# ChristianSteger/HORAYZON

Hardware: AMD Instinct MI355X
Metric: grid_cells_per_s (horizon_gridded, 360 azimuths, 3601^2 SRTM-like tile) (higher is better)
Workload: dtype f32

## Files before the change

### horayzon_amd/csrc/hz_api.hip

```cpp
#include "hz_internal.h"
#include <cmath>
#include <cstring>
#include <cstdlib>
#include <string>
#include <vector>
#include <limits>
#include <mutex>
#include <utility>
#include <thread>
#include <atomic>

namespace hz {

static thread_local std::string g_error;

int set_error(int code, const char *fmt, ...) {
    char buf[1024];
    va_list ap;
    va_start(ap, fmt);
    vsnprintf(buf, sizeof(buf), fmt, ap);
    va_end(ap);
    g_error = buf;
    return code;
}

bool is_device_ptr(const void *p) {
    if (!p) return false;
    hipPointerAttribute_t attr;
    const hipError_t e = hipPointerGetAttributes(&attr, p);
    if (e != hipSuccess) { (void)hipGetLastError(); return false; }
    return attr.type == hipMemoryTypeDevice || attr.type == hipMemoryTypeManaged;
}

template <typename T>
struct DevIn {
    const T *dev = nullptr;
    void *owned = nullptr;
    ~DevIn() { if (owned) (void)hipFree(owned); }
    int bind(const T *src, size_t count, hipStream_t st) {
        if (!src || count == 0) { dev = nullptr; return HZ_OK; }
        if (is_device_ptr(src)) { dev = src; return HZ_OK; }
        HZ_HIP(hipMalloc(&owned, count * sizeof(T)));
        HZ_HIP(hipMemcpyAsync(owned, src, count * sizeof(T), hipMemcpyHostToDevice, st));
        dev = static_cast<const T *>(owned);
        return HZ_OK;
    }
};

template <typename T>
struct DevOut {
    T *dev = nullptr;
    T *host = nullptr;
    void *owned = nullptr;
    size_t count = 0;
    ~DevOut() { if (owned) (void)hipFree(owned); }
    int bind(T *dst, size_t n) {
        count = n;
        if (!dst || n == 0) { dev = nullptr; return HZ_OK; }
        if (is_device_ptr(dst)) { dev = dst; return HZ_OK; }
        HZ_HIP(hipMalloc(&owned, n * sizeof(T)));
        dev = static_cast<T *>(owned); host = dst;
        return HZ_OK;
    }
    int finish(hipStream_t st) {
        if (host && count) HZ_HIP(hipMemcpyAsync(host, dev, count * sizeof(T), hipMemcpyDeviceToHost, st));
        return HZ_OK;
    }
};

static int select_device(int device) {
    int n = 0;
    if (hipGetDeviceCount(&n) != hipSuccess || n <= 0) {
        (void)hipGetLastError();
        return set_error(HZ_ERR_NODEV, "no HIP device available (libhorayzon_hip needs an MI355X / gfx950 GPU)");
    }
    if (device < 0 || device >= n) return set_error(HZ_ERR_ARG, "device %d out of range (%d devices)", device, n);
    HZ_HIP(hipSetDevice(device));
    return HZ_OK;
}

static inline float deg2rad_f(float ang) { return (float)(((double)ang / 180.0) * M_PI); }

struct HostTables {
    std::vector<float> azim_sin, azim_cos, elev_ang, elev_sin, elev_cos;
    std::vector<int> mid_idx;
    int elev_num = 0;
    float hori_acc = 0, low = 0, up = 0;
};

static void build_tables(int azim_num, float hori_acc_deg, float low_deg, HostTables &t) {
    float elev_ang_up_lim = 89.98;
    t.hori_acc = deg2rad_f(hori_acc_deg);
    t.low = deg2rad_f(low_deg);
    t.up = deg2rad_f(elev_ang_up_lim);
    t.azim_sin.resize((size_t)azim_num); t.azim_cos.resize((size_t)azim_num);
    float ang;
    for (int i = 0; i < azim_num; i++) {
        ang = (float)(((2 * M_PI) / azim_num) * i);
        t.azim_sin[(size_t)i] = sinf(ang);
        t.azim_cos[(size_t)i] = cosf(ang);
    }
    const double step = (double)t.hori_acc / 5.0;
    t.elev_num = (int)ceil((double)(t.up - t.low) / step) + 1;
    const size_t n = (size_t)std::max(t.elev_num, 0);
    t.elev_ang.resize(n); t.elev_sin.resize(n); t.elev_cos.resize(n);
    for (int i = 0; i < t.elev_num; i++) {
        ang = (float)((double)t.up - step * (double)i);
        t.elev_ang[(size_t)(t.elev_num - i - 1)] = ang;
        t.elev_sin[(size_t)(t.elev_num - i - 1)] = sinf(ang);
        t.elev_cos[(size_t)(t.elev_num - i - 1)] = cosf(ang);
    }
    t.mid_idx.assign(2 * (n > 0 ? n : 1), 0);
    for (int i = 0; i + 10 < t.elev_num; i++) {
        const float es = (float)((double)(t.elev_ang[(size_t)i] + t.elev_ang[(size_t)i + 10]) / 2.0);
        const int mid = (int)roundf((float)((double)(es - t.low) / step));
        t.mid_idx[2 * (size_t)i] = mid;
        const float ev = t.elev_ang[(size_t)std::min(std::max(mid, 0), t.elev_num - 1)];
        memcpy(&t.mid_idx[2 * (size_t)i + 1], &ev, sizeof(float));
    }
}

static int parse_alg(const char *s, int *alg) {
    if (s && strcmp(s, "discrete_sampling") == 0) { *alg = 0; return HZ_OK; }
    if (s && strcmp(s, "binary_search") == 0) { *alg = 1; return HZ_OK; }
    if (s && strcmp(s, "guess_constant") == 0) { *alg = 2; return HZ_OK; }
    return set_error(HZ_ERR_ARG, "invalid input argument for ray_algorithm");
}

static int check_geom(const char *s) {
    if (s && (strcmp(s, "triangle") == 0 || strcmp(s, "quad") == 0 || strcmp(s, "grid") == 0)) return HZ_OK;
    return set_error(HZ_ERR_ARG, "invalid input argument for geom_type");
}

static std::mutex g_stream_mu;
static std::vector<std::pair<int, hipStream_t>> g_stream_pool;

static int stream_acquire(int device, hipStream_t *st) {
    {
        std::lock_guard<std::mutex> lk(g_stream_mu);
        for (size_t i = 0; i < g_stream_pool.size(); i++)
            if (g_stream_pool[i].first == device) {
                *st = g_stream_pool[i].second;
                g_stream_pool.erase(g_stream_pool.begin() + (long)i);
                return HZ_OK;
            }
    }
    const hipError_t e = hipStreamCreateWithFlags(st, hipStreamNonBlocking);
    if (e != hipSuccess) return set_error(HZ_ERR_HIP, "hipStreamCreate failed: %s", hipGetErrorString(e));
    return HZ_OK;
}

static void stream_release(int device, hipStream_t st) {
    if (!st) return;
    (void)hipStreamSynchronize(st);
    std::lock_guard<std::mutex> lk(g_stream_mu);
    g_stream_pool.emplace_back(device, st);
}

static int scene_new(int device, Scene **out) {
    int rc = select_device(device);
    if (rc) return rc;
    Scene *sc = new Scene();
    sc->device = device;
    if ((rc = stream_acquire(device, &sc->stream))) { delete sc; return rc; }
    *out = sc;
    return HZ_OK;
}

static void scene_free(Scene *sc) {
    if (!sc) return;
    (void)hipSetDevice(sc->device);
    stream_release(sc->device, sc->stream);
    if (sc->near_buf) (void)hipFree(sc->near_buf);
    if (sc->left_buf) (void)hipFree(sc->left_buf);
    if (sc->owns_blob && sc->blob) (void)hipFree(sc->blob);
    delete sc;
}

struct Terrain {
    int device = 0;
    Scene *scene = nullptr;
    bool owns_scene = false;
    int offset_0 = 0, offset_1 = 0, dim_in_0 = 0, dim_in_1 = 0;
    void *tilt = nullptr, *norm = nullptr, *enl = nullptr, *elev = nullptr, *mask = nullptr;
    double *refrac_fac = nullptr;
    bool own_tilt = false, own_norm = false, own_enl = false, own_elev = false, own_mask = false;
    float fill = 0, ang_max = 89.0f;
    int refrac = 0;
    int count_work = 0;
    unsigned long long *counters = nullptr;
    float *sun_dev = nullptr;
    size_t sun_cap = 0;
    hipStream_t stream = nullptr;
    bool initialised = false;
};

static void terrain_release_arrays(Terrain *t) {
    (void)hipSetDevice(t->device);
    if (t->own_tilt && t->tilt) (void)hipFree(t->tilt);
    if (t->own_norm && t->norm) (void)hipFree(t->norm);
    if (t->own_enl && t->enl) (void)hipFree(t->enl);
    if (t->own_elev && t->elev) (void)hipFree(t->elev);
    if (t->own_mask && t->mask) (void)hipFree(t->mask);
    if (t->refrac_fac) { (void)hipFree(t->refrac_fac); t->refrac_fac = nullptr; }
    t->tilt = t->norm = t->enl = t->elev = t->mask = nullptr;
    t->own_tilt = t->own_norm = t->own_enl = t->own_elev = t->own_mask = false;
    if (t->counters) { (void)hipFree(t->counters); t->counters = nullptr; }
    if (t->sun_dev) { (void)hipFree(t->sun_dev); t->sun_dev = nullptr; t->sun_cap = 0; }
    if (t->owns_scene && t->scene) scene_free(t->scene);
    t->scene = nullptr; t->owns_scene = false; t->initialised = false;
}

static int persist(const void *src, size_t bytes, hipStream_t st, void **dst, bool *own) {
    if (is_device_ptr(src)) { *dst = const_cast<void *>(src); *own = false; return HZ_OK; }
    HZ_HIP(hipMalloc(dst, bytes ? bytes : 16));
    *own = true;
    HZ_HIP(hipMemcpyAsync(*dst, src, bytes, hipMemcpyHostToDevice, st));
    return HZ_OK;
}

struct HostPinner {
    std::vector<std::pair<char *, size_t>> regions;
    std::vector<std::pair<char *, size_t>> planned;
    std::atomic<int> done{0};
    std::atomic<bool> failed{false};
    std::thread worker;
    int device = 0;
    void start(int dev, char *base, const std::vector<size_t> &chunk_bytes) {
        device = dev;
        const uintptr_t page = 4096;
        size_t total = 0;
        for (size_t b : chunk_bytes) total += b;
        if (total < ((size_t)8 << 20)) return;
        const uintptr_t first = reinterpret_cast<uintptr_t>(base);
        const uintptr_t last_page = (first + total) & ~(page - 1);
        uintptr_t lo = (first + page - 1) & ~(page - 1);
        uintptr_t cur = first;
        for (size_t k = 0; k < chunk_bytes.size(); k++) {
            cur += chunk_bytes[k];
            const uintptr_t hi = std::min(cur & ~(page - 1), last_page);
            regions.emplace_back(reinterpret_cast<char *>(lo), hi > lo ? (size_t)(hi - lo) : 0);
            lo = std::max(lo, hi);
        }
        planned = regions;
        worker = std::thread([this]() {
            (void)hipSetDevice(device);
            for (size_t k = 0; k < regions.size(); k++) {
                if (!failed.load() && regions[k].second &&
                    hipHostRegister(regions[k].first, regions[k].second, hipHostRegisterDefault) != hipSuccess) {
                    (void)hipGetLastError();
                    regions[k].second = 0;
                    failed.store(true);
                } else if (failed.load()) {
                    regions[k].second = 0;
                }
                done.store((int)k + 1, std::memory_order_release);
            }
        });
    }
    std::vector<size_t> cuts_for(const char *dst, size_t bytes) const {
        std::vector<size_t> cuts;
        int need = 0;
        for (size_t k = 0; k < planned.size(); k++) {
            const char *lo = planned[k].first, *hi = lo + planned[k].second;
            if (planned[k].second && hi > dst && lo < dst + bytes) need = (int)k + 1;
        }
        while (done.load(std::memory_order_acquire) < need) std::this_thread::yield();
        for (int k = 0; k < need; k++) {
            const char *lo = planned[(size_t)k].first, *hi = lo + planned[(size_t)k].second;
            if (planned[(size_t)k].second == 0) continue;
            if (lo > dst && lo < dst + bytes) cuts.push_back((size_t)(lo - dst));
            if (hi > dst && hi < dst + bytes) cuts.push_back((size_t)(hi - dst));
        }
        std::sort(cuts.begin(), cuts.end());
        cuts.erase(std::unique(cuts.begin(), cuts.end()), cuts.end());
        return cuts;
    }
    void finish() {
        if (worker.joinable()) worker.join();
        for (auto &r : regions) if (r.second) (void)hipHostUnregister(r.first);
        regions.clear();
    }
    ~HostPinner() { finish(); }
};

struct NearMonitor {
    int device = 0;
    hipStream_t st_mon = nullptr;
    hipEvent_t ready = nullptr, done = nullptr;
    void *buf = nullptr;
    size_t buf_bytes = 0;
    unsigned long long *cnt = nullptr;
    bool active = false;
    int launch(const Scene *sc, const HorizonArgs &a, int n, int seed, hipStream_t st) {
        device = sc->device;
        const int nb = horizon_num_blocks(a);
        std::vector<int> pick;
        for (int b = 0; b < nb; b++) {
            uint32_t h = (uint32_t)b * 2654435761u + (uint32_t)seed * 40503u;
            h ^= h >> 15; h *= 2246822519u; h ^= h >> 13;
            if (h % (uint32_t)n == 0u) pick.push_back(b);
        }
        if (pick.empty()) return HZ_OK;
        int rc;
        if (!st_mon && (rc = stream_acquire(device, &st_mon))) return rc;
        if (!ready) { HZ_HIP(hipEventCreateWithFlags(&ready, hipEventDisableTiming)); HZ_HIP(hipEventCreateWithFlags(&done, hipEventDisableTiming)); }
        const size_t cbytes = HZ_CNT_N * sizeof(unsigned long long) + HZ_REDO_CAP * sizeof(int);
        const size_t row_bytes = ((size_t)a.azim_num * sizeof(float) + 255) & ~(size_t)255;
        const size_t need = cbytes + row_bytes + pick.size() * sizeof(int);
        if (need > buf_bytes) {
            if (buf) { (void)hipFree(buf); buf = nullptr; buf_bytes = 0; }
            HZ_HIP(hipMalloc(&buf, need + need / 4));
            buf_bytes = need + need / 4;
        }
        cnt = (unsigned long long *)buf;
        float *scratch = (float *)((char *)buf + cbytes);
        int *d_list = (int *)((char *)buf + cbytes + row_bytes);
        HZ_HIP(hipEventRecord(ready, st));
        HZ_HIP(hipStreamWaitEvent(st_mon, ready, 0));
        HZ_HIP(hipMemsetAsync(buf, 0, cbytes, st_mon));
        HZ_HIP(hipMemcpyAsync(d_list, pick.data(), pick.size() * sizeof(int), hipMemcpyHostToDevice, st_mon));
        HZ_HIP(hipStreamSynchronize(st_mon));
        HorizonArgs v = a;
        v.count_work = 1; v.verify_near = 1; v.level_stack = 1;
        v.scratch_row = scratch;
        v.counters = cnt; v.tile_list = d_list; v.n_list = (int)pick.size();
        if ((rc = horizon_launch(sc, v, st_mon, nullptr))) return rc;
        HZ_HIP(hipEventRecord(done, st_mon));
        active = true;
        return HZ_OK;
    }
    int collect(hipStream_t st, unsigned long long *verified, unsigned long long *violations) {
        unsigned long long c2[HZ_CNT_N] = {0};
        HZ_HIP(hipStreamWaitEvent(st, done, 0));
        HZ_HIP(hipMemcpyAsync(c2, cnt, sizeof(c2), hipMemcpyDeviceToHost, st_mon));
        HZ_HIP(hipStreamSynchronize(st_mon));
        *verified += c2[21]; *violations += c2[10];
        active = false;
        return HZ_OK;
    }
    ~NearMonitor() {
        if (st_mon) { (void)hipSetDevice(device); stream_release(device, st_mon); }
        if (ready) (void)hipEventDestroy(ready);
        if (done) (void)hipEventDestroy(done);
        if (buf) (void)hipFree(buf);
    }
};

static void print_near_reasons(const unsigned *near_reasons) {
    unsigned h[20] = {0};
    if (hipMemcpy(h, near_reasons, sizeof(h), hipMemcpyDeviceToHost) != hipSuccess) { (void)hipGetLastError(); return; }
    static const char *nm[14] = {"frame", "vertex_on_axis", "edge_over_axis", "az_tolerance", "inplane_edge", "crossing_near_axis",
                                 "interval", "precision", "edge_on", "orientation", "origin_below", "axis_in_triangle", "window_or_mask",
                                 "bad_mesh_nearby"};
    fprintf(stderr, "hz near reasons: cells %u certified %u", h[0], h[1]);
    for (int b = 0; b < 14; b++) if (h[2 + b]) fprintf(stderr, " %s %u", nm[b], h[2 + b]);
    fprintf(stderr, " | tasks %u bins %u\n", h[16], h[17]);
}

static void print_reference_report(const Scene *sc, int alg, unsigned long long cells, unsigned long long rays, size_t slab_cells,
                                   int dim_in_0, int dim_in_1, int azim_num, double kernel_s, bool certificates_off, bool certificates_per_cell) {
    static const char *alg_name[3] = {"discrete_sampling", "binary search", "guess horizon from previous azimuth direction"};
    printf("Horizon detection algorithm: %s\n", alg_name[alg]);
    printf("Number of grid cells for which horizon is computed: %llu \n", cells);
    printf("Fraction of total number of grid cells: %g %%\n", (double)((float)cells / (float)slab_cells * 100.0f));
    printf("Total memory required for horizon output: %g GB\n",
           (double)(((float)dim_in_0 * (float)dim_in_1 * (float)azim_num * 4.0f) / 1.0e9f));
    printf("Ray tracing time: %g s\n", kernel_s);
    printf("Number of rays shot: %llu\n", rays);
    printf("Average number of rays per location and azimuth: %.2f \n",
           cells ? (double)((float)rays / (float)(cells * (unsigned long long)azim_num)) : 0.0);
    if (certificates_off)
        printf("Near-field certificates off: a DEM quad that is not part of a height field over the (x, y) plane, or a triangle "
               "of the outer simplified domain, is too large for the per-cell guard (results unaffected, slower)\n");
    else if (certificates_per_cell)
        printf("Near-field certificates per cell: %u DEM triangle(s) project onto the (x, y) plane collapsed or against the "
               "majority, %d outer-domain triangle(s); cells near them run without (results unaffected)\n", sc->hdr.n_flipped, sc->hdr.n_tin);
    fflush(stdout);
}

static int alloc_hori_chunk(int rows_all, size_t row_bytes, bool skip_hori, int fixed_rows, int *chunk_rows_out, void **buf) {
    size_t target = skip_hori ? ((size_t)16 << 30) : ((size_t)4 << 30);
    {
        size_t free_b = 0, total_b = 0;
        if (hipMemGetInfo(&free_b, &total_b) == hipSuccess) {
            if (!skip_hori) {
                const size_t all = (size_t)rows_all * row_bytes;
                const size_t parts = std::max<size_t>(1, (all + ((size_t)8 << 30) - 1) / ((size_t)8 << 30));
                if (free_b / 6 >= all / parts + row_bytes) target = std::max(target, all / parts + row_bytes);
            }
        } else (void)hipGetLastError();
    }
    const bool fixed = fixed_rows > 0;
    for (;;) {
        int chunk_rows = rows_all;
        if (fixed) chunk_rows = std::min(chunk_rows, fixed_rows);
        else {
            chunk_rows = (int)std::max<size_t>(16, std::min<size_t>((size_t)chunk_rows, target / row_bytes));
            const int n_ch = (rows_all + chunk_rows - 1) / chunk_rows;
            chunk_rows = std::min(chunk_rows, std::max(16, ((rows_all + n_ch - 1) / n_ch + 15) / 16 * 16));
        }
        chunk_rows = std::min(chunk_rows, rows_all);
        *chunk_rows_out = chunk_rows;
        if (hipMalloc(buf, (size_t)chunk_rows * row_bytes) == hipSuccess) return HZ_OK;
        (void)hipGetLastError();
        *buf = nullptr;
        if (fixed || target <= ((size_t)1 << 30)) return set_error(HZ_ERR_HIP, "hipMalloc of the horizon chunk (%zu bytes) failed", (size_t)chunk_rows * row_bytes);
        target >>= 1;
    }
}

static int near_prepass(const Scene *sc, NearArgs &na, hipStream_t st, float *ms_near) {
    const size_t cells = (size_t)(na.row_end - na.row_begin) * na.dim_in_1;
    const size_t idx_bytes = (cells * (size_t)na.azim_num * 2 + 255) & ~(size_t)255;
    const size_t need = idx_bytes + cells * 4;
    if (sc->near_bytes < need) {
        if (sc->near_buf) (void)hipFree(sc->near_buf);
        sc->near_buf = nullptr; sc->near_bytes = 0;
        if (hipMalloc(&sc->near_buf, need) != hipSuccess) return set_error(HZ_ERR_HIP, "hipMalloc of the near-field certificates failed");
        sc->near_bytes = need;
    }
    na.near_idx = (unsigned short *)sc->near_buf;
    na.near_r = (float *)((char *)sc->near_buf + idx_bytes);
    hipEvent_t n0 = nullptr, n1 = nullptr;
    if (hipEventCreate(&n0) != hipSuccess || hipEventCreate(&n1) != hipSuccess) {
        if (n0) (void)hipEventDestroy(n0);
        return set_error(HZ_ERR_HIP, "hipEventCreate failed");
    }
    (void)hipEventRecord(n0, st);
    const int rc = near_launch(sc, na, st);
    (void)hipEventRecord(n1, st);
    if (!rc) {
        (void)hipEventSynchronize(n1);
        float mn = 0.0f;
        (void)hipEventElapsedTime(&mn, n0, n1);
        *ms_near += mn;
    }
    (void)hipEventDestroy(n0); (void)hipEventDestroy(n1);
    return rc;
}

static int plan_leftover(const Scene *sc, const hz_opts *opts, int rows_max, int dim_in_1, int left_t[HZ_LEFT_LEVELS], HorizonArgs &a) {
    int n_left_launches = 0;
    for (int l = 0; l < HZ_LEFT_LEVELS; l++) left_t[l] = 0;
    const int pack = opts ? opts->left_min : 0;
    const unsigned upack = pack == 0 ? HZ_LEFT_DEFAULT : (pack < 0 ? 0u : (unsigned)pack);
    for (int l = 0; l < HZ_LEFT_LEVELS; l++) {
        left_t[l] = (int)std::min((upack >> (8 * l)) & 0xffu, 56u);
        if (left_t[l] == 0) break;
        n_left_launches = l + 1;
    }
    if ((opts && opts->count_work) || n_left_launches == 0) return 0;
    const TileMap tm = make_tile_map((rows_max + 15) / 16, (dim_in_1 + 15) / 16);
    unsigned long long units = (unsigned long long)tm.per_xcd * 8ull * 4ull;
    unsigned long long total = 0, cap_max = 0;
    for (int l = 0; l < n_left_launches; l++) {
        unsigned long long cap = ((units * (unsigned long long)left_t[l] + 63ull) & ~63ull) + 64ull;
        if (opts && opts->left_cap_test > 0) cap = std::min<unsigned long long>(cap, ((unsigned long long)opts->left_cap_test + 63ull) & ~63ull);
        a.left_base[l] = (unsigned)total; a.left_cap[l] = (unsigned)cap;
        total += cap; cap_max = std::max(cap_max, cap);
        units = cap / 64ull;
    }
    const size_t rec_bytes = (size_t)total * HZ_LEFT_WORDS * sizeof(unsigned);
    const size_t sort_words = 4 * (size_t)cap_max + sort_temp_elems((size_t)cap_max) + 64;
    const size_t need = rec_bytes + sort_words * sizeof(uint32_t);
    if (total >= (1ull << 31) || (unsigned long long)rows_max * (unsigned long long)dim_in_1 >= 0xffffffffull) return 0;
    if (sc->left_bytes < need) {
        if (sc->left_buf) (void)hipFree(sc->left_buf);
        sc->left_buf = nullptr; sc->left_bytes = 0;
        if (hipMalloc(&sc->left_buf, need) != hipSuccess) { (void)hipGetLastError(); sc->left_buf = nullptr; return 0; }
        sc->left_bytes = need;
    }
    a.left_sort = (uint32_t *)((char *)sc->left_buf + rec_bytes); a.left_cap_max = (unsigned)cap_max;
    return n_left_launches;
}

static int horizon_run(const Scene *sc, const float *vec_norm, const float *vec_north, int offset_0,
                       int offset_1, float *hori_buffer, int dim_in_0, int dim_in_1, int azim_num,
                       float dist_search, float hori_acc, const char *ray_algorithm,
                       float elev_ang_low_lim, const uint8_t *mask, float hori_fill, float ray_org_elev,
                       const hz_opts *opts, const hz_topo_out *topo, hz_stats *stats) {
    int alg = 2;
    int rc = parse_alg(ray_algorithm, &alg);
    if (rc) return rc;
    if (!vec_norm || !vec_north || !mask) return set_error(HZ_ERR_ARG, "vec_norm, vec_north and mask must not be NULL");
    if (dim_in_0 <= 0 || dim_in_1 <= 0 || azim_num <= 0) return set_error(HZ_ERR_ARG, "dim_in_0, dim_in_1 and azim_num must be positive");
    if (offset_0 < 0 || offset_1 < 0 || offset_0 + dim_in_0 > sc->hdr.d0 || offset_1 + dim_in_1 > sc->hdr.d1)
        return set_error(HZ_ERR_ARG, "inconsistency between input arguments dem_dim_0, dem_dim_1, offset_0, offset_1 and vec_norm");
    if (!(hori_acc > 0.0f) || hori_acc > 10.0f) return set_error(HZ_ERR_ARG, "limit of hori_acc (10 degree) is exceeded");
    const bool skip_hori = opts && opts->skip_hori;
    if (!hori_buffer && !skip_hori) return set_error(HZ_ERR_ARG, "hori_buffer is NULL");
    if (opts && opts->svf && !opts->vec_tilt) return set_error(HZ_ERR_ARG, "opts.svf needs opts.vec_tilt");
    if (opts && opts->svf && azim_num < 2) return set_error(HZ_ERR_ARG, "opts.svf needs azim_num >= 2");
    if (topo && topo->size != (int32_t)sizeof(hz_topo_out))
        return set_error(HZ_ERR_ARG, "topo.size is %d, expected sizeof(hz_topo_out) = %d", topo->size, (int)sizeof(hz_topo_out));
    const bool want_vsf = topo && topo->vsf, want_open = topo && topo->openness;
    if (want_vsf && !(opts && opts->vec_tilt)) return set_error(HZ_ERR_ARG, "topo.vsf needs opts.vec_tilt");
    if (want_vsf && azim_num < 2) return set_error(HZ_ERR_ARG, "topo.vsf needs azim_num >= 2");
    int row_begin = 0, row_end = dim_in_0;
    if (opts && !(opts->row_begin == 0 && opts->row_end == 0)) {
        row_begin = opts->row_begin;
        row_end = (opts->row_end == -1) ? dim_in_0 : opts->row_end;
        if (row_begin < 0 || row_end < 0 || row_end > dim_in_0 || row_begin > row_end)
            return set_error(HZ_ERR_ARG, "invalid row slab [%d, %d) for dim_in_0 = %d", opts->row_begin, opts->row_end, dim_in_0);
        if (row_begin == row_end) return HZ_OK;
    }
    HZ_HIP(hipSetDevice(sc->device));
    std::lock_guard<std::mutex> run_lock(sc->run_mu);
    hipStream_t st = sc->stream;
    Timer t_total; t_total.start();

    HostTables tb;
    build_tables(azim_num, hori_acc, elev_ang_low_lim, tb);
    if (tb.elev_num < 2) return set_error(HZ_ERR_ARG, "elevation table is empty (elev_ang_low_lim too high)");
    const float dist_m = (float)((double)dist_search * 1000.0);

    const size_t ncell = (size_t)dim_in_0 * dim_in_1;
    const size_t slab_cells = (size_t)(row_end - row_begin) * dim_in_1;
    Timer t_h2d; t_h2d.start();
    DevIn<float> d_norm, d_north, d_tilt, d_as, d_ac, d_ea, d_es, d_ec;
    DevIn<int> d_mid;
    DevIn<uint8_t> d_mask;
    const bool inputs_are_slab = opts && opts->inputs_are_slab;
    const size_t in_off = (size_t)row_begin * dim_in_1;
    const size_t src_off = inputs_are_slab ? 0 : in_off;
    (void)ncell;
    if ((rc = d_norm.bind(vec_norm + 3 * src_off, slab_cells * 3, st))) return rc;
    if ((rc = d_north.bind(vec_north + 3 * src_off, slab_cells * 3, st))) return rc;
    if ((rc = d_mask.bind(mask + src_off, slab_cells, st))) return rc;
    if ((opts && opts->svf) || want_vsf) if ((rc = d_tilt.bind(opts->vec_tilt + 3 * src_off, slab_cells * 3, st))) return rc;
    const float *norm0 = d_norm.dev - 3 * in_off, *north0 = d_north.dev - 3 * in_off;
    const uint8_t *mask0 = d_mask.dev - in_off;
    const float *tilt0 = d_tilt.dev ? d_tilt.dev - 3 * in_off : nullptr;
    if ((rc = d_as.bind(tb.azim_sin.data(), (size_t)azim_num, st))) return rc;
    if ((rc = d_ac.bind(tb.azim_cos.data(), (size_t)azim_num, st))) return rc;
    if ((rc = d_ea.bind(tb.elev_ang.data(), (size_t)tb.elev_num, st))) return rc;
    if ((rc = d_es.bind(tb.elev_sin.data(), (size_t)tb.elev_num, st))) return rc;
    if ((rc = d_ec.bind(tb.elev_cos.data(), (size_t)tb.elev_num, st))) return rc;
    if ((rc = d_mid.bind(tb.mid_idx.data(), tb.mid_idx.size(), st))) return rc;
    DevOut<float> d_hori, d_svf, d_vsf, d_open;
    DevIn<float> d_azim;
    const bool want_svf = opts && opts->svf;
    const bool want_topo = want_svf || want_vsf || want_open;
    const bool hori_is_slab = opts && opts->hori_is_slab;
    float *hori_slab_host = hori_buffer ? (hori_is_slab ? hori_buffer : hori_buffer + (size_t)row_begin * dim_in_1 * azim_num) : nullptr;
    float *hori_row0 = hori_slab_host ? hori_slab_host - (size_t)row_begin * dim_in_1 * azim_num : nullptr;
    float *svf_slab = want_svf ? (hori_is_slab ? opts->svf : opts->svf + (size_t)row_begin * dim_in_1) : nullptr;
    if ((rc = d_svf.bind(svf_slab, svf_slab ? slab_cells : 0))) return rc;
    float *vsf_slab = want_vsf ? (hori_is_slab ? topo->vsf : topo->vsf + (size_t)row_begin * dim_in_1) : nullptr;
    float *open_slab = want_open ? (hori_is_slab ? topo->openness : topo->openness + (size_t)row_begin * dim_in_1) : nullptr;
    if ((rc = d_vsf.bind(vsf_slab, vsf_slab ? slab_cells : 0))) return rc;
    if ((rc = d_open.bind(open_slab, open_slab ? slab_cells : 0))) return rc;
    int chunk_rows = row_end - row_begin;
    void *tmp_hori = nullptr, *tmp_hori2 = nullptr;
    size_t tmp_bytes = 0;
    struct TmpFree { void **p; ~TmpFree() { if (*p) (void)hipFree(*p); } } tmp_free{&tmp_hori}, tmp_free2{&tmp_hori2};
    const size_t row_bytes = (size_t)dim_in_1 * azim_num * 4;
    const bool stream_out = !skip_hori && !is_device_ptr(hori_slab_host);
    if (skip_hori || stream_out) {
        if (skip_hori && !want_topo) return set_error(HZ_ERR_ARG, "skip_hori without svf, vsf or openness: nothing to compute");
        if ((rc = alloc_hori_chunk(row_end - row_begin, row_bytes, skip_hori, (opts && opts->chunk_rows > 0) ? opts->chunk_rows : 0, &chunk_rows, &tmp_hori)))
            return rc;
        tmp_bytes = (size_t)chunk_rows * row_bytes;
        if (stream_out && chunk_rows < row_end - row_begin) { HZ_HIP(hipMalloc(&tmp_hori2, (size_t)chunk_rows * row_bytes)); tmp_bytes *= 2; }
    } else {
        if ((rc = d_hori.bind(hori_slab_host, slab_cells * (size_t)azim_num))) return rc;
    }
    std::vector<float> azim_h;
    if (want_topo) {
        azim_h.resize((size_t)azim_num);
        for (int i = 0; i < azim_num; i++) azim_h[(size_t)i] = (float)(((2 * M_PI) / azim_num) * i);
        if ((rc = d_azim.bind(azim_h.data(), (size_t)azim_num, st))) return rc;
    }
    DevIn<unsigned long long> d_cnt;
    unsigned long long zeros[HZ_CNT_N] = {0};
    void *cnt_dev = nullptr;
    HZ_HIP(hipMalloc(&cnt_dev, sizeof(zeros) + 2 * HZ_REDO_CAP * sizeof(int)));
    d_cnt.owned = cnt_dev;
    HZ_HIP(hipStreamSynchronize(st));
    const double h2d_s = t_h2d.stop();

    HorizonArgs a;
    a.vec_norm = norm0; a.vec_north = north0; a.mask = mask0;
    a.offset_0 = offset_0; a.offset_1 = offset_1; a.dim_in_0 = dim_in_0; a.dim_in_1 = dim_in_1;
    a.azim_num = azim_num; a.elev_num = tb.elev_num; a.alg = alg;
    a.hori_acc = tb.hori_acc; a.low = tb.low; a.up = tb.up; a.dist = dist_m;
    a.hori_fill = hori_fill; a.ray_org_elev = ray_org_elev;
    a.azim_sin = d_as.dev; a.azim_cos = d_ac.dev; a.elev_ang = d_ea.dev; a.elev_sin = d_es.dev; a.elev_cos = d_ec.dev;
    a.mid_idx = d_mid.dev;
    a.top_nodes = opts ? opts->top_nodes : -1;
    a.regroup = opts ? opts->regroup : -1;
    a.count_work = opts ? opts->count_work : 0;
    a.hit_cache = (opts && opts->no_hit_cache) ? 0 : 1;
    a.counters = (unsigned long long *)cnt_dev;
    const int near_opt = opts ? opts->no_near_skip : 0;
    const bool height_field = (sc->hdr.flags & HZ_BLOB_HEIGHT_FIELD) != 0;
    const bool bad_map = (sc->hdr.flags & HZ_BLOB_BAD_MAP) != 0;
    const bool use_near = near_opt <= 0 && (height_field || bad_map || near_opt < 0) &&
                          azim_num <= near_max_azim() && tb.elev_num <= 65534;
    a.near_idx = nullptr; a.near_r = nullptr; a.scratch_row = nullptr;
    a.tile_list = nullptr; a.n_list = 0;
    const int verify_n = (opts && opts->verify_near > 0) ? opts->verify_near : 0;
    a.verify_near = (opts && opts->count_work) ? verify_n : 0;
    float ms_near = 0.0f;

    unsigned long long cnt[16] = {0}, n_verified = 0, n_mon_violations = 0;
    NearMonitor mon;
    float ms = 0.0f, ms_svf = 0.0f;
    int fallbacks = 0;
    unsigned long long redo_blocks = 0, redo_groups = 0;

    struct Ev { hipEvent_t a = nullptr, b = nullptr, c = nullptr, d = nullptr, l = nullptr; };
    std::vector<Ev> evs;
    std::vector<size_t> ev_of;
    hipStream_t st_copy = nullptr;
    auto free_events = [&]() {
        for (auto &e : evs) {
            if (e.a) (void)hipEventDestroy(e.a);
            if (e.b) (void)hipEventDestroy(e.b);
            if (e.c) (void)hipEventDestroy(e.c);
            if (e.d) (void)hipEventDestroy(e.d);
            if (e.l) (void)hipEventDestroy(e.l);
        }
        if (st_copy) { stream_release(sc->device, st_copy); st_copy = nullptr; }
    };
    if (stream_out && (rc = stream_acquire(sc->device, &st_copy))) return rc;
    if (use_near) {
        const size_t cells = (size_t)std::min(chunk_rows, row_end - row_begin) * dim_in_1;
        const size_t need = ((cells * (size_t)azim_num * 2 + 255) & ~(size_t)255) + cells * 4;
        if (sc->near_bytes < need) {
            if (sc->near_buf) (void)hipFree(sc->near_buf);
            sc->near_buf = nullptr; sc->near_bytes = 0;
            if (hipMalloc(&sc->near_buf, need) != hipSuccess) { free_events(); return set_error(HZ_ERR_HIP, "hipMalloc of the near-field certificates failed"); }
            sc->near_bytes = need;
        }
    }
    int left_t[HZ_LEFT_LEVELS];
    const int n_left_launches = plan_leftover(sc, opts, std::min(chunk_rows, row_end - row_begin), dim_in_1, left_t, a);
    a.left_min = n_left_launches > 0 ? left_t[0] : 0;
    a.left_rec = n_left_launches > 0 ? (unsigned *)sc->left_buf : nullptr;
    a.left_regroup = (opts && (opts->left_tune & 0xff) > 0) ? (opts->left_tune & 0xff) : HZ_LEFT_REGROUP;
    a.left_key_shift = (opts && ((opts->left_tune >> 8) & 0xff) > 0) ? std::min(((opts->left_tune >> 8) & 0xff) - 1, 8) : HZ_LEFT_KEY_SHIFT;
    a.persist_grid = (opts && opts->persist_grid > 0) ? opts->persist_grid : 0;
    a.no_persist = (opts && opts->persist_grid < 0) ? 1 : 0;
    unsigned *near_reasons = nullptr;
    struct ReasonsFree { unsigned **p; ~ReasonsFree() { if (*p) (void)hipFree(*p); } } reasons_free{&near_reasons};
    if (use_near && opts && opts->verbose >= 2) {
        if (hipMalloc((void **)&near_reasons, 20 * sizeof(unsigned)) != hipSuccess) { (void)hipGetLastError(); near_reasons = nullptr; }
        else (void)hipMemsetAsync(near_reasons, 0, 20 * sizeof(unsigned), st);
    }
    HostPinner pinner;
    if (stream_out && !(opts && opts->no_host_pin)) {
        std::vector<size_t> cb;
        for (int rb = row_begin; rb < row_end; rb += chunk_rows) cb.push_back((size_t)(std::min(rb + chunk_rows, row_end) - rb) * row_bytes);
        pinner.start(sc->device, reinterpret_cast<char *>(hori_slab_host), cb);
    }
    auto copy_out = [&](int k) -> int {
        const int rb = row_begin + k * chunk_rows, re = std::min(rb + chunk_rows, row_end);
        const void *src = (k & 1) ? tmp_hori2 : tmp_hori;
        Ev &e = evs[ev_of[(size_t)k]];
        char *dst = reinterpret_cast<char *>(hori_row0 + (size_t)rb * dim_in_1 * azim_num);
        const size_t bytes = (size_t)(re - rb) * row_bytes;
        std::vector<size_t> cuts;
        if (!pinner.planned.empty()) cuts = pinner.cuts_for(dst, bytes);
        cuts.push_back(bytes);
        if (hipStreamWaitEvent(st_copy, e.c, 0) != hipSuccess)
            return set_error(HZ_ERR_HIP, "copy of the horizon chunk failed: %s", hipGetErrorString(hipGetLastError()));
        size_t from = 0;
        for (size_t to : cuts) {
            if (to > from && hipMemcpyAsync(dst + from, static_cast<const char *>(src) + from, to - from, hipMemcpyDeviceToHost, st_copy) != hipSuccess)
                return set_error(HZ_ERR_HIP, "copy of the horizon chunk failed: %s", hipGetErrorString(hipGetLastError()));
            from = to;
        }
        if (hipEventRecord(e.d, st_copy) != hipSuccess)
            return set_error(HZ_ERR_HIP, "copy of the horizon chunk failed: %s", hipGetErrorString(hipGetLastError()));
        return HZ_OK;
    };
    auto fail = [&](int code) { (void)hipStreamSynchronize(st); if (st_copy) (void)hipStreamSynchronize(st_copy); free_events(); return code; };
    int n_chunk = 0;
    unsigned long long left_cells = 0, left_again = 0;
    float ms_left = 0.0f;
    for (int rb = row_begin; rb < row_end; rb += chunk_rows, n_chunk++) {
        const int re = std::min(rb + chunk_rows, row_end);
        float *hori_chunk;
        if (stream_out) hori_chunk = (float *)((n_chunk & 1) ? tmp_hori2 : tmp_hori);
        else if (skip_hori) hori_chunk = (float *)tmp_hori;
        else hori_chunk = d_hori.dev + (size_t)(rb - row_begin) * dim_in_1 * azim_num;
        a.hori = hori_chunk - (size_t)rb * dim_in_1 * azim_num;
        a.row_begin = rb; a.row_end = re;
        if (use_near) {
            NearArgs na;
            na.vec_norm = norm0; na.vec_north = north0; na.mask = mask0;
            na.azim_sin = d_as.dev; na.azim_cos = d_ac.dev;
            na.offset_0 = offset_0; na.offset_1 = offset_1; na.dim_in_1 = dim_in_1; na.row_begin = rb; na.row_end = re;
            na.azim_num = azim_num; na.elev_num = tb.elev_num;
            na.ray_org_elev = ray_org_elev; na.hori_acc = tb.hori_acc; na.low = tb.low; na.up = tb.up;
            na.reasons = near_reasons;
            na.ignore_bad_map = near_opt < 0 ? 1 : 0;
            if ((rc = near_prepass(sc, na, st, &ms_near))) return fail(rc);
            a.near_idx = na.near_idx; a.near_r = na.near_r;
        }
        {
            Ev e;
            if (hipEventCreate(&e.a) != hipSuccess || hipEventCreate(&e.b) != hipSuccess || hipEventCreate(&e.c) != hipSuccess ||
                hipEventCreate(&e.d) != hipSuccess) {
                evs.push_back(e);
                return fail(set_error(HZ_ERR_HIP, "hipEventCreate failed"));
            }
            evs.push_back(e);
            ev_of.push_back(evs.size() - 1);
            if (hipMemcpyAsync(cnt_dev, zeros, sizeof(zeros), hipMemcpyHostToDevice, st) != hipSuccess)
                return fail(set_error(HZ_ERR_HIP, "counter reset failed"));
            if (stream_out && n_chunk >= 2) (void)hipStreamWaitEvent(st, evs[ev_of[(size_t)n_chunk - 2]].d, 0);
            a.level_stack = (sc->level_stack.load(std::memory_order_relaxed) != 0 || (opts && opts->level_stack > 0)) ? 1
                            : ((opts && opts->level_stack < 0) ? opts->level_stack : 0);
            (void)hipEventRecord(e.a, st);
            if (verify_n > 0 && !a.count_work && use_near) {
                if ((rc = mon.launch(sc, a, verify_n, rb, st))) return fail(rc);
            }
            auto launch_chunk = [&](int *safe_out) -> int {
                int r = horizon_launch(sc, a, st, safe_out);
                if (r || n_left_launches == 0) return r;
                if (!evs.back().l && hipEventCreate(&evs.back().l) != hipSuccess) return set_error(HZ_ERR_HIP, "hipEventCreate failed");
                (void)hipEventRecord(evs.back().l, st);
                for (int l = 1; l <= n_left_launches && !r; l++) {
                    if ((r = left_sort(a, l - 1, st))) break;
                    HorizonArgs b = a;
                    b.left_mode = l; b.left_min = l < n_left_launches ? left_t[l] : 0;
                    if (n_left_launches > 1) b.level_stack = 1;
                    b.tile_list = nullptr; b.n_list = 0;
                    r = horizon_launch(sc, b, st, nullptr);
                }
                return r;
            };
            int safe = 0;
            rc = launch_chunk(&safe);
            if (!rc && !safe) {
                unsigned long long cov[32] = {0};
                if (hipMemcpyAsync(cov, cnt_dev, sizeof(cov), hipMemcpyDeviceToHost, st) != hipSuccess ||
                    hipStreamSynchronize(st) != hipSuccess)
                    return fail(set_error(HZ_ERR_HIP, "horizon kernel failed: %s", hipGetErrorString(hipGetLastError())));
                const unsigned long long ov = cov[8], lov = cov[30];
                if (ov != 0 || lov != 0) {
                    const unsigned long long tiles = (unsigned long long)((re - rb + 7) / 8) * (unsigned long long)((dim_in_1 + 7) / 8);
                    fallbacks++;
                    a.level_stack = 1;
                    if (ov <= HZ_REDO_CAP && lov <= HZ_REDO_CAP && (ov + lov) * 4 <= tiles) {
                        redo_blocks += ov + lov; redo_groups += lov;
                        if (ov != 0) {
                            a.tile_list = reinterpret_cast<const int *>((unsigned long long *)cnt_dev + HZ_CNT_N);
                            a.n_list = (int)ov;
                            rc = horizon_launch(sc, a, st, &safe);
                            a.tile_list = nullptr; a.n_list = 0;
                        }
                        if (!rc && lov != 0) {
                            HorizonArgs b = a;
                            b.left_mode = 1; b.left_min = 0;
                            b.tile_list = reinterpret_cast<const int *>((unsigned long long *)cnt_dev + HZ_CNT_N) + HZ_REDO_CAP;
                            b.n_list = (int)lov;
                            rc = horizon_launch(sc, b, st, nullptr);
                        }
                    } else {
                        sc->level_stack.store(1, std::memory_order_relaxed);
                        if (hipMemcpyAsync(cnt_dev, zeros, sizeof(zeros), hipMemcpyHostToDevice, st) != hipSuccess)
                            return fail(set_error(HZ_ERR_HIP, "counter reset failed"));
                        (void)hipEventRecord(e.a, st);
                        rc = launch_chunk(&safe);
                    }
                }
            }
            if (!rc && mon.active) rc = mon.collect(st, &n_verified, &n_mon_violations);
            (void)hipEventRecord(e.b, st);
            if (!rc && want_topo) {
                const size_t o = (size_t)(rb - row_begin) * dim_in_1;
                const float *tilt_chunk = tilt0 ? tilt0 + 3 * (size_t)rb * dim_in_1 : nullptr;
                if (!want_vsf && !want_open)
                    rc = svf_launch(d_azim.dev, hori_chunk, tilt_chunk, re - rb, dim_in_1, azim_num, d_svf.dev + o, st);
                else
                    rc = topo_multi_launch(d_azim.dev, hori_chunk, tilt_chunk, re - rb, dim_in_1, azim_num,
                                           want_svf ? d_svf.dev + o : nullptr, want_vsf ? d_vsf.dev + o : nullptr,
                                           want_open ? d_open.dev + o : nullptr, st);
            }
            (void)hipEventRecord(e.c, st);
            if (!rc && stream_out && n_chunk >= 1) rc = copy_out(n_chunk - 1);
            if (rc) return fail(rc);
            unsigned long long c[HZ_CNT_N];
            if (hipMemcpyAsync(c, cnt_dev, sizeof(c), hipMemcpyDeviceToHost, st) != hipSuccess ||
                hipStreamSynchronize(st) != hipSuccess)
                return fail(set_error(HZ_ERR_HIP, "horizon kernel failed: %s", hipGetErrorString(hipGetLastError())));
            float m1 = 0.0f, m2 = 0.0f;
            (void)hipEventElapsedTime(&m1, e.a, e.b);
            (void)hipEventElapsedTime(&m2, e.b, e.c);
            ms += m1; ms_svf += m2;
            if (evs.back().l) { float m3 = 0.0f; (void)hipEventElapsedTime(&m3, evs.back().l, e.b); ms_left += m3; }
            for (int k = 0; k < 16; k++) cnt[k] += c[k];
            left_cells += c[28]; left_again += c[29];
            n_verified += c[21];
            if (a.count_work && opts && opts->verbose >= 3) {
                const unsigned long long t0 = ~c[20];
                fprintf(stderr, "hz xcd spans [ms] rows %d..%d:", rb, re);
                for (int x = 0; x < 8; x++) fprintf(stderr, " %.1f", c[12 + x] ? (double)(c[12 + x] - t0) * 1.0e-5 : 0.0);
                fprintf(stderr, "\n");
            }
        }
    }
    Timer t_d2h; t_d2h.start();
    if (stream_out) {
        rc = copy_out(n_chunk - 1);
        const hipError_t se = hipStreamSynchronize(st_copy);
        pinner.finish();
        if (!rc && se != hipSuccess) rc = set_error(HZ_ERR_HIP, "copy of the horizon failed: %s", hipGetErrorString(se));
        if (rc) { free_events(); return rc; }
    }
    free_events();
    HZ_HIP(hipGetLastError());
    if ((rc = d_hori.finish(st))) return rc;
    if ((rc = d_svf.finish(st))) return rc;
    if ((rc = d_vsf.finish(st))) return rc;
    if ((rc = d_open.finish(st))) return rc;
    HZ_HIP(hipStreamSynchronize(st));
    const double d2h_s = t_d2h.stop();

    if (stats) {
        stats->num_rays += cnt[0]; stats->guard_events += cnt[1];
        stats->nodes_visited += cnt[2]; stats->tris_tested += cnt[3]; stats->num_cells += cnt[4];
        stats->wave_node_iters += cnt[5]; stats->wave_leaf_iters += cnt[6]; stats->wave_refills += cnt[7];
        stats->t_h2d_s += h2d_s; stats->t_kernel_s += (double)ms * 1e-3; stats->t_svf_s += (double)ms_svf * 1e-3;
        stats->t_d2h_s += d2h_s;
        stats->t_total_s += t_total.stop();
        stats->elev_num = tb.elev_num; stats->bvh_height = sc->hdr.height; stats->scene_bytes = sc->hdr.total_bytes;
        stats->stack_fallbacks += (uint64_t)fallbacks; stats->stack_redo_blocks += redo_blocks; stats->left_redo_groups += redo_groups;
        stats->rays_shortened += cnt[9]; stats->near_violations += cnt[10] + n_mon_violations; stats->t_near_s += (double)ms_near * 1e-3;
        stats->guard_cells += cnt[11]; stats->near_verified += n_verified;
        stats->t_left_s += (double)ms_left * 1e-3; stats->left_cells += left_cells; stats->left_again += left_again;
        stats->scratch_bytes = (uint64_t)((use_near ? sc->near_bytes : 0) + (n_left_launches > 0 ? sc->left_bytes : 0) + tmp_bytes);
        stats->height_field = height_field ? 1 : 0; stats->near_used = use_near ? 1 : 0;
    }
    if (near_reasons) print_near_reasons(near_reasons);
    if (opts && opts->verbose)
        print_reference_report(sc, alg, cnt[4], cnt[0], slab_cells, dim_in_0, dim_in_1, azim_num, (double)ms * 1e-3,
                               !use_near && near_opt <= 0 && !height_field && !bad_map, use_near && bad_map);
    return HZ_OK;
}

static int locations_run(const Scene *sc, const float *coords, const float *vec_norm, const float *vec_north,
                         float *hori_buffer, float *hori_dist_buffer, int num_loc, int azim_num,
                         float dist_search, float hori_acc, const char *ray_algorithm, float elev_ang_low_lim,
                         const float *ray_org_elev, int hori_dist_out, const hz_opts *opts, hz_stats *stats) {
    int alg = 1;
    int rc = parse_alg(ray_algorithm, &alg);
    if (rc) return rc;
    if (hori_dist_out && alg == 2)
        return set_error(HZ_ERR_ARG, "horizon detection algorithm 'guess_constant' not implemented for horizon "
                                     "distance computation");
    if (!coords || !vec_norm || !vec_north || !ray_org_elev || !hori_buffer) return set_error(HZ_ERR_ARG, "NULL argument");
    if (hori_dist_out && !hori_dist_buffer) return set_error(HZ_ERR_ARG, "hori_dist_buffer is NULL");
    if (num_loc <= 0 || azim_num <= 0) return set_error(HZ_ERR_ARG, "num_loc and azim_num must be positive");
    if (!(hori_acc > 0.0f) || hori_acc > 10.0f) return set_error(HZ_ERR_ARG, "limit of hori_acc (10 degree) is exceeded");
    HZ_HIP(hipSetDevice(sc->device));
    std::lock_guard<std::mutex> run_lock(sc->run_mu);
    hipStream_t st = sc->stream;
    Timer t_total; t_total.start();
    HostTables tb;
    build_tables(azim_num, hori_acc, elev_ang_low_lim, tb);
    if (tb.elev_num < 2) return set_error(HZ_ERR_ARG, "elevation table is empty (elev_ang_low_lim too high)");
    Timer t_h2d; t_h2d.start();
    DevIn<float> d_co, d_norm, d_north, d_roe, d_as, d_ac, d_ea, d_es, d_ec;
    DevIn<int> d_mid;
    const size_t n = (size_t)num_loc;
    if ((rc = d_co.bind(coords, n * 3, st))) return rc;
    if ((rc = d_norm.bind(vec_norm, n * 3, st))) return rc;
    if ((rc = d_north.bind(vec_north, n * 3, st))) return rc;
    if ((rc = d_roe.bind(ray_org_elev, n, st))) return rc;
    if ((rc = d_as.bind(tb.azim_sin.data(), (size_t)azim_num, st))) return rc;
    if ((rc = d_ac.bind(tb.azim_cos.data(), (size_t)azim_num, st))) return rc;
    if ((rc = d_ea.bind(tb.elev_ang.data(), (size_t)tb.elev_num, st))) return rc;
    if ((rc = d_es.bind(tb.elev_sin.data(), (size_t)tb.elev_num, st))) return rc;
    if ((rc = d_ec.bind(tb.elev_cos.data(), (size_t)tb.elev_num, st))) return rc;
    if ((rc = d_mid.bind(tb.mid_idx.data(), tb.mid_idx.size(), st))) return rc;
    DevOut<float> d_hori, d_dist;
    if ((rc = d_hori.bind(hori_buffer, n * (size_t)azim_num))) return rc;
    if (d_hori.host) HZ_HIP(hipMemcpyAsync(d_hori.dev, hori_buffer, n * (size_t)azim_num * 4, hipMemcpyHostToDevice, st));
    if (hori_dist_out) {
        if ((rc = d_dist.bind(hori_dist_buffer, n * (size_t)azim_num))) return rc;
        if (d_dist.host) HZ_HIP(hipMemcpyAsync(d_dist.dev, hori_dist_buffer, n * (size_t)azim_num * 4, hipMemcpyHostToDevice, st));
    }
    DevIn<unsigned long long> d_cnt;
    unsigned long long zeros[8] = {0, 0, 0, 0, 0, 0, 0, 0};
    void *cnt_dev = nullptr;
    HZ_HIP(hipMalloc(&cnt_dev, sizeof(zeros)));
    d_cnt.owned = cnt_dev;
    HZ_HIP(hipMemcpyAsync(cnt_dev, zeros, sizeof(zeros), hipMemcpyHostToDevice, st));
    HZ_HIP(hipStreamSynchronize(st));
    const double h2d_s = t_h2d.stop();

    LocationsArgs a;
    a.coords = d_co.dev; a.vec_norm = d_norm.dev; a.vec_north = d_north.dev; a.ray_org_elev = d_roe.dev;
    a.hori = d_hori.dev; a.dist = d_dist.dev;
    a.num_loc = num_loc; a.azim_num = azim_num; a.elev_num = tb.elev_num; a.alg = alg; a.hori_dist_out = hori_dist_out;
    a.hori_acc = tb.hori_acc; a.low = tb.low; a.up = tb.up; a.dist_m = (float)((double)dist_search * 1000.0);
    a.azim_sin = d_as.dev; a.azim_cos = d_ac.dev; a.elev_ang = d_ea.dev; a.elev_sin = d_es.dev; a.elev_cos = d_ec.dev;
    a.mid_idx = d_mid.dev;
    a.counters = (unsigned long long *)cnt_dev;
    hipEvent_t e0, e1;
    HZ_HIP(hipEventCreate(&e0)); HZ_HIP(hipEventCreate(&e1));
    (void)hipEventRecord(e0, st);
    rc = locations_launch(sc, a, st);
    (void)hipEventRecord(e1, st);
    const hipError_t se = hipStreamSynchronize(st);
    float ms = 0.0f;
    (void)hipEventElapsedTime(&ms, e0, e1);
    (void)hipEventDestroy(e0); (void)hipEventDestroy(e1);
// ... 199 lines not shown
    if (!scene) return set_error(HZ_ERR_ARG, "scene is NULL");
    return locations_run(reinterpret_cast<const Scene *>(scene), coords, vec_norm, vec_north, hori_buffer,
                         hori_dist_buffer, num_loc, azim_num, dist_search, hori_acc, ray_algorithm,
                         elev_ang_low_lim, ray_org_elev, hori_dist_out, opts, stats);
}

int hz_horizon_locations(const float *vert_grid, int dem_dim_0, int dem_dim_1, const float *coords,
                         const float *vec_norm, const float *vec_north, float *hori_buffer,
                         float *hori_dist_buffer, int num_loc, int azim_num, float dist_search, float hori_acc,
                         const char *ray_algorithm, const char *geom_type, float elev_ang_low_lim,
                         const float *ray_org_elev, int hori_dist_out, const hz_opts *opts, hz_stats *stats) {
    Timer t; t.start();
    hz_scene *scene = nullptr;
    hz_stats local;
    memset(&local, 0, sizeof(local));
    int rc = hz_scene_create(vert_grid, dem_dim_0, dem_dim_1, geom_type, nullptr, 0, nullptr, 0,
                             opts ? opts->device : 0, &scene, &local);
    if (rc) return rc;
    rc = hz_horizon_locations_scene(scene, coords, vec_norm, vec_north, hori_buffer, hori_dist_buffer, num_loc,
                                    azim_num, dist_search, hori_acc, ray_algorithm, elev_ang_low_lim, ray_org_elev,
                                    hori_dist_out, opts, &local);
    hz_scene_destroy(scene);
    local.t_total_s = t.stop();
    if (stats) *stats = local;
    return rc;
}

int hz_horizon_tables(int azim_num, float hori_acc, float elev_ang_low_lim, float *azim_sin,
                      float *azim_cos, int elev_cap, float *elev_ang, float *elev_sin, float *elev_cos,
                      int *elev_num) {
    if (azim_num <= 0 || !(hori_acc > 0.0f)) return set_error(HZ_ERR_ARG, "azim_num and hori_acc must be positive");
    HostTables t;
    build_tables(azim_num, hori_acc, elev_ang_low_lim, t);
    if (elev_num) *elev_num = t.elev_num;
    if (azim_sin) memcpy(azim_sin, t.azim_sin.data(), sizeof(float) * (size_t)azim_num);
    if (azim_cos) memcpy(azim_cos, t.azim_cos.data(), sizeof(float) * (size_t)azim_num);
    if (elev_ang && elev_sin && elev_cos && t.elev_num > 0 && t.elev_num <= elev_cap) {
        memcpy(elev_ang, t.elev_ang.data(), sizeof(float) * (size_t)t.elev_num);
        memcpy(elev_sin, t.elev_sin.data(), sizeof(float) * (size_t)t.elev_num);
        memcpy(elev_cos, t.elev_cos.data(), sizeof(float) * (size_t)t.elev_num);
    }
    return HZ_OK;
}

static int topo_api(int kind, const float *azim, const float *hori, const float *vec_tilt, int len_0, int len_1,
                    int len_2, float *out, int device) {
    if (!azim || !hori || !out || (kind != 2 && !vec_tilt)) return set_error(HZ_ERR_ARG, "NULL argument");
    if (len_0 <= 0 || len_1 <= 0 || len_2 < (kind == 2 ? 1 : 2)) return set_error(HZ_ERR_ARG, "Inconsistent/incorrect shapes of input arrays");
    int rc = select_device(device);
    if (rc) return rc;
    hipStream_t st = nullptr;
    const size_t ncell = (size_t)len_0 * len_1;
    DevIn<float> d_azim, d_hori, d_tilt;
    DevOut<float> d_out;
    if ((rc = d_azim.bind(azim, (size_t)len_2, st))) return rc;
    if ((rc = d_hori.bind(hori, ncell * (size_t)len_2, st))) return rc;
    if (kind != 2) if ((rc = d_tilt.bind(vec_tilt, ncell * 3, st))) return rc;
    if ((rc = d_out.bind(out, ncell))) return rc;
    if ((rc = topo_launch(kind, d_azim.dev, d_hori.dev, d_tilt.dev, len_0, len_1, len_2, d_out.dev, st))) return rc;
    if ((rc = d_out.finish(st))) return rc;
    HZ_HIP(hipStreamSynchronize(st));
    return HZ_OK;
}

int hz_sky_view_factor(const float *azim, const float *hori, const float *vec_tilt, int len_0, int len_1,
                       int len_2, float *svf, int device) {
    return topo_api(0, azim, hori, vec_tilt, len_0, len_1, len_2, svf, device);
}
int hz_visible_sky_fraction(const float *azim, const float *hori, const float *vec_tilt, int len_0, int len_1,
                            int len_2, float *vsf, int device) {
    return topo_api(1, azim, hori, vec_tilt, len_0, len_1, len_2, vsf, device);
}
int hz_topographic_openness(const float *azim, const float *hori, int len_0, int len_1, int len_2, float *top,
                            int device) {
    return topo_api(2, azim, hori, nullptr, len_0, len_1, len_2, top, device);
}

int hz_topo_params(const float *azim, const float *hori, const float *vec_tilt, int len_0, int len_1, int len_2,
                   float *svf, float *vsf, float *openness, int device) {
    const bool tilt = svf || vsf;
    if (!svf && !vsf && !openness) return set_error(HZ_ERR_ARG, "no output requested (svf, vsf and openness are NULL)");
    if (!azim || !hori || (tilt && !vec_tilt)) return set_error(HZ_ERR_ARG, "NULL argument");
    if (len_0 <= 0 || len_1 <= 0 || len_2 < (tilt ? 2 : 1)) return set_error(HZ_ERR_ARG, "Inconsistent/incorrect shapes of input arrays");
    int rc = select_device(device);
    if (rc) return rc;
    hipStream_t st = nullptr;
    const size_t ncell = (size_t)len_0 * len_1;
    DevIn<float> d_azim, d_hori, d_tilt;
    DevOut<float> d_svf, d_vsf, d_open;
    if ((rc = d_azim.bind(azim, (size_t)len_2, st))) return rc;
    if ((rc = d_hori.bind(hori, ncell * (size_t)len_2, st))) return rc;
    if (tilt) if ((rc = d_tilt.bind(vec_tilt, ncell * 3, st))) return rc;
    if ((rc = d_svf.bind(svf, svf ? ncell : 0))) return rc;
    if ((rc = d_vsf.bind(vsf, vsf ? ncell : 0))) return rc;
    if ((rc = d_open.bind(openness, openness ? ncell : 0))) return rc;
    if ((rc = topo_multi_launch(d_azim.dev, d_hori.dev, d_tilt.dev, len_0, len_1, len_2, d_svf.dev, d_vsf.dev, d_open.dev, st)))
        return rc;
    if ((rc = d_svf.finish(st)) || (rc = d_vsf.finish(st)) || (rc = d_open.finish(st))) return rc;
    HZ_HIP(hipStreamSynchronize(st));
    return HZ_OK;
}

int hz_debug_sort_pairs(uint32_t *keys, uint32_t *vals, size_t n, int device) {
    if (!keys || !vals) return set_error(HZ_ERR_ARG, "NULL argument");
    int rc = select_device(device);
    if (rc) return rc;
    hipStream_t st = nullptr;
    void *dk = nullptr, *dv = nullptr, *dk2 = nullptr, *dv2 = nullptr, *tmp = nullptr;
    const size_t bytes = (n ? n : 1) * 4;
    HZ_HIP(hipMalloc(&dk, bytes)); HZ_HIP(hipMalloc(&dv, bytes)); HZ_HIP(hipMalloc(&dk2, bytes)); HZ_HIP(hipMalloc(&dv2, bytes));
    HZ_HIP(hipMalloc(&tmp, sort_temp_elems(n) * 4 + 16));
    HZ_HIP(hipMemcpy(dk, keys, n * 4, hipMemcpyHostToDevice));
    HZ_HIP(hipMemcpy(dv, vals, n * 4, hipMemcpyHostToDevice));
    rc = radix_sort_pairs_u32((uint32_t *)dk, (uint32_t *)dv, (uint32_t *)dk2, (uint32_t *)dv2, n, (uint32_t *)tmp, st);
    if (!rc) {
        HZ_HIP(hipStreamSynchronize(st));
        HZ_HIP(hipMemcpy(keys, dk, n * 4, hipMemcpyDeviceToHost));
        HZ_HIP(hipMemcpy(vals, dv, n * 4, hipMemcpyDeviceToHost));
    }
    (void)hipFree(dk); (void)hipFree(dv); (void)hipFree(dk2); (void)hipFree(dv2); (void)hipFree(tmp);
    return rc;
}

int hz_debug_exclusive_scan(const uint32_t *in, uint32_t *out, size_t n, int device) {
    if (!in || !out) return set_error(HZ_ERR_ARG, "NULL argument");
    int rc = select_device(device);
    if (rc) return rc;
    hipStream_t st = nullptr;
    void *di = nullptr, *dout = nullptr, *tmp = nullptr;
    const size_t bytes = (n ? n : 1) * 4;
    HZ_HIP(hipMalloc(&di, bytes)); HZ_HIP(hipMalloc(&dout, bytes)); HZ_HIP(hipMalloc(&tmp, scan_temp_elems(n) * 4 + 16));
    HZ_HIP(hipMemcpy(di, in, n * 4, hipMemcpyHostToDevice));
    rc = exclusive_scan_u32((const uint32_t *)di, (uint32_t *)dout, n, (uint32_t *)tmp, st);
    if (!rc) {
        HZ_HIP(hipStreamSynchronize(st));
        HZ_HIP(hipMemcpy(out, dout, n * 4, hipMemcpyDeviceToHost));
    }
    (void)hipFree(di); (void)hipFree(dout); (void)hipFree(tmp);
    return rc;
}

int hz_debug_valu_peak(int device, int packed, int waves_per_simd, double *winst_per_s_per_simd,
                       double *clock_ghz, int *simds) {
    int rc = select_device(device);
    if (rc) return rc;
    return bench_valu_peak(packed, waves_per_simd, winst_per_s_per_simd, clock_ghz, simds);
}

int hz_debug_set(const char *key, int value) {
    if (!key) return hz::set_error(HZ_ERR_ARG, "hz_debug_set: null key");
    if (!strcmp(key, "shadow_fast_cap")) hz::g_shadow_fast_cap.store(value < 0 ? HZ_SHADOW_FAST_CAP_DEFAULT : value, std::memory_order_relaxed);
    else if (!strcmp(key, "topo_wide")) hz::g_topo_wide.store(value != 0, std::memory_order_relaxed);
    else if (!strcmp(key, "accum_chunk")) hz::g_accum_chunk.store(value < 0 ? 0 : value, std::memory_order_relaxed);
    else return hz::set_error(HZ_ERR_ARG, "hz_debug_set: unknown key '%s'", key);
    return HZ_OK;
}

int hz_debug_inst_rate(int device, int op, double *cycles_per_inst) {
    int rc = select_device(device);
    if (rc) return rc;
    return bench_inst_rate(op, cycles_per_inst);
}

int hz_debug_copy_peak(int device, size_t bytes, double *gbs) {
    int rc = select_device(device);
    if (rc) return rc;
    return bench_copy_peak(bytes, gbs);
}

static int slope_api(int which, const float *x, const float *y, const float *z, int len_0, int len_1,
                     const float *rot_mat, int output_rot, float *vec_tilt, int device) {
    if (!x || !y || !z || !vec_tilt) return set_error(HZ_ERR_ARG, "NULL argument");
    if (len_0 <= 0 || len_1 <= 0) return set_error(HZ_ERR_ARG, "Inconsistent shapes / number of dimensions of input arrays");
    if (which == 1 && output_rot && !rot_mat) return set_error(HZ_ERR_ARG, "'rot_mat' must be provided for 'output_rot = True'");
    int rc = select_device(device);
    if (rc) return rc;
    hipStream_t st = nullptr;
    const size_t n = (size_t)len_0 * len_1;
    DevIn<float> dx, dy, dz, dr;
    DevOut<float> dt;
    if ((rc = dx.bind(x, n, st))) return rc;
    if ((rc = dy.bind(y, n, st))) return rc;
    if ((rc = dz.bind(z, n, st))) return rc;
    if ((rc = dr.bind(rot_mat, rot_mat ? n * 9 : 0, st))) return rc;
    if ((rc = dt.bind(vec_tilt, n * 3))) return rc;
    if ((rc = prep_slope(which, dx.dev, dy.dev, dz.dev, len_0, len_1, dr.dev, output_rot, dt.dev, st))) return rc;
    if ((rc = dt.finish(st))) return rc;
    HZ_HIP(hipStreamSynchronize(st));
    return HZ_OK;
}

int hz_slope_plane_meth(const float *x, const float *y, const float *z, int len_0, int len_1,
                        const float *rot_mat, int output_rot, float *vec_tilt, int device) {
    return slope_api(0, x, y, z, len_0, len_1, rot_mat, output_rot, vec_tilt, device);
}
int hz_slope_vector_meth(const float *x, const float *y, const float *z, int len_0, int len_1,
                         const float *rot_mat, int output_rot, float *vec_tilt, int device) {
    return slope_api(1, x, y, z, len_0, len_1, rot_mat, output_rot, vec_tilt, device);
}

static int check_ellps(int ellps) {
    if (ellps < 0 || ellps > 2) return set_error(HZ_ERR_ARG, "Unknown value for 'ellps'");
    return HZ_OK;
}

int hz_lonlat2ecef(const double *lon, const double *lat, const float *h, size_t n, int ellps, double *x_ecef,
                   double *y_ecef, double *z_ecef, int device) {
    if (!lon || !lat || !h || !x_ecef || !y_ecef || !z_ecef) return set_error(HZ_ERR_ARG, "NULL argument");
    int rc = check_ellps(ellps);
    if (rc) return rc;
    if ((rc = select_device(device))) return rc;
    hipStream_t st = nullptr;
    DevIn<double> dlon, dlat; DevIn<float> dh; DevOut<double> ox, oy, oz;
    if ((rc = dlon.bind(lon, n, st)) || (rc = dlat.bind(lat, n, st)) || (rc = dh.bind(h, n, st))) return rc;
    if ((rc = ox.bind(x_ecef, n)) || (rc = oy.bind(y_ecef, n)) || (rc = oz.bind(z_ecef, n))) return rc;
    if ((rc = prep_lonlat2ecef(ellps, dlon.dev, dlat.dev, dh.dev, n, ox.dev, oy.dev, oz.dev, st))) return rc;
    if ((rc = ox.finish(st)) || (rc = oy.finish(st)) || (rc = oz.finish(st))) return rc;
    HZ_HIP(hipStreamSynchronize(st));
    return HZ_OK;
}

int hz_wgs2swiss(const double *lon, const double *lat, const float *h_wgs, size_t n, double *e, double *no, float *h_ch,
                 int device) {
    if (!lon || !lat || !h_wgs || !e || !no || !h_ch) return set_error(HZ_ERR_ARG, "NULL argument");
    int rc = select_device(device);
    if (rc) return rc;
    hipStream_t st = nullptr;
    DevIn<double> da, db; DevIn<float> dh; DevOut<double> oa, ob; DevOut<float> oh;
    if ((rc = da.bind(lon, n, st)) || (rc = db.bind(lat, n, st)) || (rc = dh.bind(h_wgs, n, st))) return rc;
    if ((rc = oa.bind(e, n)) || (rc = ob.bind(no, n)) || (rc = oh.bind(h_ch, n))) return rc;
    if ((rc = prep_wgs2swiss(da.dev, db.dev, dh.dev, n, oa.dev, ob.dev, oh.dev, st))) return rc;
    if ((rc = oa.finish(st)) || (rc = ob.finish(st)) || (rc = oh.finish(st))) return rc;
    HZ_HIP(hipStreamSynchronize(st));
    return HZ_OK;
}

int hz_swiss2wgs(const double *e, const double *no, const float *h_ch, size_t n, double *lon, double *lat, float *h_wgs,
                 int device) {
    if (!e || !no || !h_ch || !lon || !lat || !h_wgs) return set_error(HZ_ERR_ARG, "NULL argument");
    int rc = select_device(device);
    if (rc) return rc;
    hipStream_t st = nullptr;
    DevIn<double> da, db; DevIn<float> dh; DevOut<double> oa, ob; DevOut<float> oh;
    if ((rc = da.bind(e, n, st)) || (rc = db.bind(no, n, st)) || (rc = dh.bind(h_ch, n, st))) return rc;
    if ((rc = oa.bind(lon, n)) || (rc = ob.bind(lat, n)) || (rc = oh.bind(h_wgs, n))) return rc;
    if ((rc = prep_swiss2wgs(da.dev, db.dev, dh.dev, n, oa.dev, ob.dev, oh.dev, st))) return rc;
    if ((rc = oa.finish(st)) || (rc = ob.finish(st)) || (rc = oh.finish(st))) return rc;
    HZ_HIP(hipStreamSynchronize(st));
    return HZ_OK;
}

int hz_ecef2enu(const double *x_ecef, const double *y_ecef, const double *z_ecef, size_t n, double lon_or,
                double lat_or, int ellps, float *x_enu, float *y_enu, float *z_enu, int device) {
    if (!x_ecef || !y_ecef || !z_ecef || !x_enu || !y_enu || !z_enu) return set_error(HZ_ERR_ARG, "NULL argument");
    if (lon_or < -180.0 || lon_or > 180.0) return set_error(HZ_ERR_ARG, "Value for 'lon_or' is outside of valid range");
    if (lat_or < -90.0 || lat_or > 90.0) return set_error(HZ_ERR_ARG, "Value for 'lat_or' is outside of valid range");
    int rc = check_ellps(ellps);
    if (rc) return rc;
    if ((rc = select_device(device))) return rc;
    hipStream_t st = nullptr;
    DevIn<double> dx, dy, dz; DevOut<float> ox, oy, oz;
    if ((rc = dx.bind(x_ecef, n, st)) || (rc = dy.bind(y_ecef, n, st)) || (rc = dz.bind(z_ecef, n, st))) return rc;
    if ((rc = ox.bind(x_enu, n)) || (rc = oy.bind(y_enu, n)) || (rc = oz.bind(z_enu, n))) return rc;
    if ((rc = prep_ecef2enu(ellps, lon_or, lat_or, dx.dev, dy.dev, dz.dev, n, ox.dev, oy.dev, oz.dev, st))) return rc;
    if ((rc = ox.finish(st)) || (rc = oy.finish(st)) || (rc = oz.finish(st))) return rc;
    HZ_HIP(hipStreamSynchronize(st));
    return HZ_OK;
}

int hz_ecef2enu_vector(const float *vec_ecef, size_t n, double lon_or, double lat_or, int ellps, float *vec_enu,
                       int device) {
    if (!vec_ecef || !vec_enu) return set_error(HZ_ERR_ARG, "NULL argument");
    int rc = check_ellps(ellps);
    if (rc) return rc;
    if ((rc = select_device(device))) return rc;
    hipStream_t st = nullptr;
    DevIn<float> dv; DevOut<float> dout;
    if ((rc = dv.bind(vec_ecef, n * 3, st)) || (rc = dout.bind(vec_enu, n * 3))) return rc;
    if ((rc = prep_ecef2enu_vector(ellps, lon_or, lat_or, dv.dev, n, dout.dev, st))) return rc;
    if ((rc = dout.finish(st))) return rc;
    HZ_HIP(hipStreamSynchronize(st));
    return HZ_OK;
}

int hz_surf_norm(const double *lon, const double *lat, size_t n, float *vec_norm_ecef, int device) {
    if (!lon || !lat || !vec_norm_ecef) return set_error(HZ_ERR_ARG, "NULL argument");
    int rc = select_device(device);
    if (rc) return rc;
    hipStream_t st = nullptr;
    DevIn<double> dlon, dlat; DevOut<float> dout;
    if ((rc = dlon.bind(lon, n, st)) || (rc = dlat.bind(lat, n, st)) || (rc = dout.bind(vec_norm_ecef, n * 3))) return rc;
    if ((rc = prep_surf_norm(dlon.dev, dlat.dev, n, dout.dev, st))) return rc;
    if ((rc = dout.finish(st))) return rc;
    HZ_HIP(hipStreamSynchronize(st));
    return HZ_OK;
}

int hz_north_dir(const double *x_ecef, const double *y_ecef, const double *z_ecef, const float *vec_norm_ecef,
                 size_t n, int ellps, float *vec_north_ecef, int device) {
    if (!x_ecef || !y_ecef || !z_ecef || !vec_norm_ecef || !vec_north_ecef) return set_error(HZ_ERR_ARG, "NULL argument");
    int rc = check_ellps(ellps);
    if (rc) return rc;
    if ((rc = select_device(device))) return rc;
    hipStream_t st = nullptr;
    DevIn<double> dx, dy, dz; DevIn<float> dn; DevOut<float> dout;
    if ((rc = dx.bind(x_ecef, n, st)) || (rc = dy.bind(y_ecef, n, st)) || (rc = dz.bind(z_ecef, n, st))) return rc;
// ... 413 lines not shown
```

### horayzon_amd/csrc/hz_horizon.hip

```cpp
#include "hz_search.h"
#include <vector>

namespace hz {

#ifndef HZ_TPB
#define HZ_TPB 256
#endif
#define HZ_WPB (HZ_TPB / 64)
#ifndef HZ_QLEN
#define HZ_QLEN 2
#endif

struct HorizonParams {
    SceneView sv;
    Tables tb;
    const float *vec_norm, *vec_north;
    const uint8_t *mask;
    float *hori;
    int offset_0, offset_1, dim_in_1;
    int row_begin, row_end;
    TileMap tm;
    float dist, hori_fill, ray_org_elev;
    float dist_box, neg_tau;
    int top_nodes, regroup, stack_bytes, leaf_bias, stage_bytes, hit_cache, stack_cap;
    int pre_bytes;
    const unsigned short *near_idx;
    const float *near_r;
    float *scratch_row;
    int verify_near;
    unsigned verify_mask;
    unsigned long long *counters;
    const int *tile_list;
    int n_list;
    int *redo_list;
    int left_min, left_mode;
    unsigned left_in_base;
    unsigned left_out_base, left_out_cap;
    unsigned *left_rec, *left_in_ctl, *left_out_ctl;
    const unsigned *left_perm;
    int persist;
    unsigned *queue;
};

__device__ __forceinline__ void hz_left_write(unsigned *w, unsigned cert, unsigned k, unsigned flags,
                                                        unsigned ind, unsigned prev, unsigned pazim, unsigned count, float lim_up, float lim_low,
                                                        float elev_samp, float ev, unsigned cache, float st0, float st1, float st2) {
    w[0] = cert;
    w[1] = k; w[2] = flags; w[3] = ind; w[4] = prev; w[5] = pazim; w[6] = count;
    w[7] = __float_as_uint(lim_up); w[8] = __float_as_uint(lim_low); w[9] = __float_as_uint(elev_samp); w[10] = __float_as_uint(ev);
    w[11] = cache; w[12] = __float_as_uint(st0); w[13] = __float_as_uint(st1); w[14] = __float_as_uint(st2); w[15] = 0u;
}

template <int ALG, bool COUNT, bool STAGE, bool NODELET, bool LEVELSTACK, bool LEFT = false>
#ifndef HZ_WG_PER_CU
#define HZ_WG_PER_CU 5
#endif
__global__ __launch_bounds__(HZ_TPB, (COUNT ? 4 : HZ_WG_PER_CU) * (4 / HZ_WPB)) void k_horizon(HorizonParams p_arg) {
    typedef const __attribute__((address_space(4))) HorizonParams *hz_kparams;
    hz_kparams pk = (hz_kparams)__builtin_amdgcn_kernarg_segment_ptr();
#if defined(__HIP_DEVICE_COMPILE__)
#define HZ_LOAD_PARAMS(dst) dst = *pk
#else
#define HZ_LOAD_PARAMS(dst) dst = p_arg
#endif
    HorizonParams p;
    HZ_LOAD_PARAMS(p);
    extern __shared__ __attribute__((aligned(16))) unsigned char smem[];
    int *stack = reinterpret_cast<int *>(smem + p.pre_bytes);
    const float4 *top = reinterpret_cast<const float4 *>(smem + p.pre_bytes + p.stack_bytes);
    const int tid = threadIdx.x;
    const int ntop = p.top_nodes;
    if (NODELET && ntop > 0) {
        float4 *dst = reinterpret_cast<float4 *>(smem + p.pre_bytes + p.stack_bytes);
        const float4 *src = reinterpret_cast<const float4 *>(p.sv.nodes);
        for (int i = tid; i < ntop * 2; i += HZ_TPB) dst[i] = src[i];
        __syncthreads();
    }

    const int wave = __builtin_amdgcn_readfirstlane(tid >> 6);
    const int xcc_own = (int)(__builtin_amdgcn_s_getreg((3 << 11) | 20) & 7u);
    int xcc_off = 0;
    int left_on = 1;
  for (;;) {
    asm volatile("" : "+s"(pk));
    HZ_LOAD_PARAMS(p);
    int tid_b = tid;
    asm volatile("" : "+v"(tid_b));
    const int lane = tid_b & 63;
#define HZ_KEEP(x) asm volatile("" : "+s"(x))
    HZ_KEEP(p.leaf_bias); HZ_KEEP(p.regroup); HZ_KEEP(p.neg_tau); HZ_KEEP(p.sv.cx); HZ_KEEP(p.sv.cy); HZ_KEEP(p.sv.cz);
    HZ_KEEP(p.near_idx); HZ_KEEP(p.near_r);
#undef HZ_KEEP
    int ti = 0, tj = 0;
    int blk = (int)blockIdx.x * HZ_WPB + wave;
    unsigned rec0 = 0u, rec_n = 0u;
    if (LEFT) {
        blk = -1;
        const unsigned groups = (p.left_in_ctl[1] + 63u) / 64u;
        if (p.tile_list) {
            const int b = (int)blockIdx.x * HZ_WPB + wave;
            const int g = b < p.n_list ? p.tile_list[b] : -1;
            if (g >= 0 && (unsigned)g < groups) { blk = g; rec0 = (unsigned)g * 64u; rec_n = min(64u, p.left_in_ctl[1] - (unsigned)g * 64u); }
        } else
        while (xcc_off < 8) {
            const unsigned x = (unsigned)((xcc_own + xcc_off) & 7);
            unsigned q = 0u;
            if (lane == 0) q = atomicAdd(&p.left_in_ctl[8 + x], 1u);
            q = (unsigned)__builtin_amdgcn_readfirstlane((int)q);
            const unsigned g = (((q >> 5) * 8u + x) << 5) | (q & 31u);
            if (g < groups) { blk = (int)g; rec0 = g * 64u; rec_n = min(64u, p.left_in_ctl[1] - g * 64u); break; }
            xcc_off++;
        }
        if (blk < 0) break;
    } else if (p.persist) {
        blk = -1;
        while (xcc_off < 8) {
            const int x = (xcc_own + xcc_off) & 7;
            int q = 0;
            if (lane == 0) q = (int)atomicAdd(&p.queue[x], 1u);
            q = __builtin_amdgcn_readfirstlane(q);
            if (q < p.tm.per_xcd * 4) { blk = (((q >> 2) * 8 + x) << 2) | (q & 3); break; }
            xcc_off++;
        }
        if (blk < 0) break;
    } else if (p.tile_list) blk = (blk < p.n_list) ? p.tile_list[blk] : -1;
    else if (HZ_WPB != 4) {
        const int b = (int)blockIdx.x, x = b & 7, t = b >> 3, per = 4 / HZ_WPB;
        blk = (((t / per) * 8 + x) * 4) + (t % per) * HZ_WPB + wave;
    }
    blk = __builtin_amdgcn_readfirstlane(blk);
    bool has_tile = blk >= 0 && (LEFT || hz_tile_of_block(p.tm, blk >> 2, &ti, &tj));
    int i = p.row_begin + ti * 16 + ((blk >> 1) & 1) * 8 + (lane >> 3);
    int j = tj * 16 + (blk & 1) * 8 + (lane & 7);
    const unsigned *rec = nullptr;
    if (LEFT) {
        has_tile = (unsigned)lane < rec_n;
        if (has_tile) {
            rec = p.left_rec + ((size_t)p.left_in_base + (size_t)p.left_perm[rec0 + (unsigned)lane]) * HZ_LEFT_WORDS;
            const unsigned c0 = rec[0];
            has_tile = c0 != 0xffffffffu;
            const unsigned di = c0 / (unsigned)p.dim_in_1;
            i = p.row_begin + (int)di; j = (int)(c0 - di * (unsigned)p.dim_in_1);
        }
    }
    const bool in_dom = has_tile && (i < p.row_end) && (j < p.dim_in_1);

    const Tables &t = p.tb;
    const unsigned long long t_start = COUNT ? (unsigned long long)wall_clock64() : 0ull;
    const size_t cell = in_dom ? ((size_t)i * p.dim_in_1 + j) : 0;
    bool done = !in_dom;
    const unsigned cert = in_dom ? (unsigned)(i - p.row_begin) * (unsigned)p.dim_in_1 + (unsigned)j : 0u;
    const bool to_scratch = COUNT && p.scratch_row != nullptr;
    float *const hori0 = to_scratch ? p.scratch_row : p.hori + (size_t)p.row_begin * p.dim_in_1 * (size_t)t.azim_num;
    const unsigned cell_stride = to_scratch ? 0u : 1u;
    Sink out;
    out.hori = COUNT ? hori0 + (size_t)(cert * cell_stride) * (size_t)t.azim_num : hori0 + (size_t)cert * (size_t)t.azim_num;
    out.dist = nullptr; out.dist_hit = 0.0f;
    out.stage = reinterpret_cast<float *>(smem) + tid_b;
    out.stride = HZ_TPB;
    float ox = 0, oy = 0, oz = 0;
    float r01 = 0, r02 = 0, r11 = 0, r12 = 0, r21 = 0, r22 = 0;
    const bool masked = in_dom && p.mask[cell] != 1;
    {
        unsigned long long m = __ballot(masked);
        while (m) {
            const int src = __ffsll((long long)m) - 1;
            m &= m - 1;
            float *row = COUNT ? hori0 + (size_t)((unsigned)__shfl((int)cert, src) * cell_stride) * (size_t)t.azim_num
                               : hori0 + (size_t)__shfl((int)cert, src) * (size_t)t.azim_num;
            for (int k = lane; k < t.azim_num; k += 64) row[k] = p.hori_fill;
        }
    }
    if (in_dom) {
        if (masked) {
            done = true;
        } else {
            const float norm_x = p.vec_norm[3 * cell], norm_y = p.vec_norm[3 * cell + 1], norm_z = p.vec_norm[3 * cell + 2];
            const float north_x = p.vec_north[3 * cell], north_y = p.vec_north[3 * cell + 1], north_z = p.vec_north[3 * cell + 2];
            const float *v = p.sv.verts + 3 * ((size_t)(i + p.offset_0) * p.sv.d1 + (size_t)(j + p.offset_1));
            ox = v[0] + norm_x * p.ray_org_elev;
            oy = v[1] + norm_y * p.ray_org_elev;
            oz = v[2] + norm_z * p.ray_org_elev;
            r01 = north_x; r02 = norm_x;
            r11 = north_y; r12 = norm_y;
            r21 = north_z; r22 = norm_z;
        }
    }
#define HZ_OC(ocx, ocy, ocz) float ocx, ocy, ocz; { float ax_ = ox, ay_ = oy, az_ = oz; \
        asm volatile("" : "+v"(ax_), "+v"(ay_), "+v"(az_)); \
        ocx = ax_ - p.sv.cx; ocy = ay_ - p.sv.cy; ocz = az_ - p.sv.cz; }
    const float tfar = p.dist;

    Search s;
    s.k = 0; s.phase = PH_NEWAZ; s.ind = 0; s.prev = 0; s.pazim = 0; s.count = 0;
    s.lim_up = 0; s.lim_low = 0; s.elev_samp = 0; s.ev = 0;
    unsigned rays = 0, guards = 0, w_adv = 0;
    TravCounters tc; tc.nodes = 0; tc.tris = 0; tc.w_nodes = 0; tc.w_leaves = 0;
    const unsigned cells_cnt = (in_dom && !done && !LEFT) ? 1u : 0u;
    bool ray_active = false, last_hit = false;
    float dx = 0, dy = 0, dz = 1;
    RayBox rb = hz_raybox(0, 0, 0, 0, 0, 1);
    TravState ts; hz_trav_reset(ts);
    int cache = 0;
    bool second = false;
    bool overflow = false;
    unsigned shortened = 0;
    unsigned w_verified = 0, w_violations = 0;
    bool verifying = false, first_result = false, want_v = false;
    float tn = 0.0f;
    bool had_guard = false;
    if (LEFT && !done) {
        s.k = (int)rec[1]; s.phase = (int)(rec[2] & 0xffu); s.ind = (int)rec[3]; s.prev = (int)rec[4]; s.pazim = (int)rec[5]; s.count = (int)rec[6];
        s.lim_up = __uint_as_float(rec[7]); s.lim_low = __uint_as_float(rec[8]); s.elev_samp = __uint_as_float(rec[9]); s.ev = __uint_as_float(rec[10]);
        cache = (int)rec[11];
        last_hit = (rec[2] & 0x100u) != 0u;
        had_guard = (rec[2] & 0x400u) != 0u;
        if (STAGE) { out.stage[0] = __uint_as_float(rec[12]); out.stage[out.stride] = __uint_as_float(rec[13]); out.stage[2 * out.stride] = __uint_as_float(rec[14]); }
        if (rec[2] & 0x200u) {
            const float ec = t.elev_cos[s.ind], es = t.elev_sin[s.ind];
            const float rx = ec * t.azim_sin[s.k], ry = ec * t.azim_cos[s.k], rz = es;
            const float r00 = r11 * r22 - r21 * r12, r10 = r21 * r02 - r01 * r22, r20 = r01 * r12 - r11 * r02;
            dx = (r00 * rx + r01 * ry) + r02 * rz;
            dy = (r10 * rx + r11 * ry) + r12 * rz;
            dz = (r20 * rx + r21 * ry) + r22 * rz;
            HZ_OC(ocx, ocy, ocz)
            rb = hz_raybox(ocx + p.neg_tau * dx, ocy + p.neg_tau * dy, ocz + p.neg_tau * dz, dx, dy, dz);
            hz_trav_reset(ts);
            ray_active = true;
        }
    }

    int left_min = (COUNT || !left_on || __popcll(__ballot(!done)) <= p.left_min + 8) ? 0 : p.left_min;
    while (__ballot(!done) != 0ull) {
        if (!COUNT && left_min > 0 && __popcll(__ballot(!done)) <= left_min) {
            const unsigned long long um = __ballot(!done);
            if (um != 0ull && !(!LEVELSTACK && __ballot(overflow) != 0ull)) {
                const unsigned n = (unsigned)__popcll(um);
                unsigned *const out_rec = p.left_rec + (size_t)p.left_out_base * HZ_LEFT_WORDS;
                unsigned base = 0u;
                if (lane == 0) base = atomicAdd(&p.left_out_ctl[0], n);
                base = (unsigned)__builtin_amdgcn_readfirstlane((int)base);
                if (base + n > p.left_out_cap) {
                    left_on = 0; left_min = 0;
                    if (base + (unsigned)lane < p.left_out_cap) out_rec[(size_t)(base + (unsigned)lane) * HZ_LEFT_WORDS] = 0xffffffffu;
                } else {
                    if (lane == 0) atomicAdd(&p.counters[LEFT ? 29 : 28], (unsigned long long)n);
                    if (!done) {
                        const unsigned rank = (unsigned)__builtin_amdgcn_mbcnt_hi((unsigned)(um >> 32), __builtin_amdgcn_mbcnt_lo((unsigned)um, 0u));
                        const unsigned flags = (unsigned)s.phase | (last_hit ? 0x100u : 0u) | (ray_active ? 0x200u : 0u) | ((guards != 0u || had_guard) ? 0x400u : 0u);
                        hz_left_write(out_rec + (size_t)(base + rank) * HZ_LEFT_WORDS, cert, (unsigned)s.k, flags,
                                      (unsigned)s.ind, (unsigned)s.prev, (unsigned)s.pazim, (unsigned)s.count, s.lim_up, s.lim_low, s.elev_samp, s.ev, (unsigned)cache,
                                      STAGE ? out.stage[0] : 0.0f, STAGE ? out.stage[out.stride] : 0.0f, STAGE ? out.stage[2 * out.stride] : 0.0f);
                        done = true;
                    }
                }
            }
        }

        if (__ballot(!done) == 0ull) break;
        if (!done && !ray_active) {
            if (COUNT) HZ_WAVE_TICK(w_adv, lane);
            unsigned cert_r = cert;
            asm volatile("" : "+v"(cert_r));
            out.hori = COUNT ? hori0 + (size_t)(cert_r * cell_stride) * (size_t)t.azim_num : hori0 + (size_t)cert_r * (size_t)t.azim_num;
            if (advance<ALG, STAGE>(s, last_hit, t, out, guards)) {
                const float ec = t.elev_cos[s.ind], es = t.elev_sin[s.ind];
                const float asn = t.azim_sin[s.k], acs = t.azim_cos[s.k];
                int near_i = 0x7fffffff;
                float near_rad = 0.0f;
                if (p.near_idx != nullptr) {
                    near_i = (int)p.near_idx[(size_t)cert_r * (size_t)t.azim_num + s.k];
                    near_rad = p.near_r[cert_r];
                }
                const float rx = ec * asn, ry = ec * acs, rz = es;
                float nx_ = r01, ny_ = r11, nz_ = r21;
                asm volatile("" : "+v"(nx_), "+v"(ny_), "+v"(nz_));
                const float r00 = ny_ * r22 - nz_ * r12;
                const float r10 = nz_ * r02 - nx_ * r22;
                const float r20 = nx_ * r12 - ny_ * r02;
                dx = (r00 * rx + r01 * ry) + r02 * rz;
                dy = (r10 * rx + r11 * ry) + r12 * rz;
                dz = (r20 * rx + r21 * ry) + r22 * rz;
                    tn = (s.ind >= near_i) ? near_rad : p.neg_tau;
                if (COUNT && tn > 0.0f) shortened++;
                if (COUNT) want_v = p.verify_near && tn > 0.0f && (((rays + cert) & p.verify_mask) == 0u);
                HZ_OC(ocx, ocy, ocz)
                rb = hz_raybox(ocx + tn * dx, ocy + tn * dy, ocz + tn * dz, dx, dy, dz);
                hz_trav_reset(ts);
                second = p.hit_cache && (cache != 0) && (s.ind <= s.pazim) && (s.k > 0);
                if (second) {
                    ts.node = cache;
                    if (!LEVELSTACK) { ts.sp = 1; stack[HZ_TPB + tid] = 0; second = false; }
                }
                ray_active = true;
                rays++;
            } else {
                done = true;
            }
        }
        bool start_v = false, viol = false;
        if (ray_active) {
            int r;
            r = hz_trace<HZ_TPB, COUNT, HZ_QLEN, NODELET, LEVELSTACK>(p.sv.nodes, p.sv.prims, top, ntop, stack, tid, ox, oy, oz,
                                                 dx, dy, dz, tfar, p.dist_box, rb, ts, p.regroup, p.leaf_bias, tc, p.stack_cap, overflow);
            if (r == 0 && second) {
                second = false; hz_trav_reset(ts);
            } else if (COUNT && want_v && r != 2) {
                want_v = false; verifying = true; first_result = (r == 1); start_v = true;
                HZ_OC(ocx, ocy, ocz)
                rb = hz_raybox(ocx + p.neg_tau * dx, ocy + p.neg_tau * dy, ocz + p.neg_tau * dz, dx, dy, dz);
                hz_trav_reset(ts);
            } else if (r != 2) {
                if (COUNT && verifying) { viol = ((r == 1) != first_result); verifying = false; }
                ray_active = false; last_hit = (r == 1);
                if (r == 1) cache = p.sv.anc[HZ_LEAF_ID(ts.lq0)];
            }
        }
        if (COUNT) {
            w_verified += (unsigned)__popcll(__ballot(start_v));
            w_violations += (unsigned)__popcll(__ballot(viol));
        }
    }
    unsigned long long r = rays, g = guards, nc = tc.nodes, tcn = tc.tris, cc = cells_cnt;
    unsigned long long wn = tc.w_nodes, wl = tc.w_leaves, wa = w_adv;
    for (int off = 32; off > 0; off >>= 1) {
        r += __shfl_xor(r, off); g += __shfl_xor(g, off); cc += __shfl_xor(cc, off);
        if (COUNT) {
            nc += __shfl_xor(nc, off); tcn += __shfl_xor(tcn, off);
            wn += __shfl_xor(wn, off); wl += __shfl_xor(wl, off); wa += __shfl_xor(wa, off);
        }
    }
    const bool wave_overflowed = !LEVELSTACK && __ballot(overflow) != 0ull;
    if (wave_overflowed) {
        if (lane == 0) {
            const unsigned long long slot = atomicAdd(&p.counters[LEFT ? 30 : 8], 1ull);
            if (slot < (unsigned long long)HZ_REDO_CAP) p.redo_list[(LEFT ? HZ_REDO_CAP : 0) + (int)slot] = blk;
        }
    } else {
    const int guard_cells = __popcll(__ballot(guards != 0u && !(LEFT && had_guard)));
    if (lane == 0) {
        if (r) atomicAdd(&p.counters[0], r);
        if (g) { atomicAdd(&p.counters[1], g); atomicAdd(&p.counters[11], (unsigned long long)guard_cells); }
        if (cc) atomicAdd(&p.counters[4], cc);
        if (COUNT) {
            atomicAdd(&p.counters[2], nc); atomicAdd(&p.counters[3], tcn);
            atomicAdd(&p.counters[5], wn); atomicAdd(&p.counters[6], wl); atomicAdd(&p.counters[7], wa);
        }
    }
    if (COUNT) {
        if (lane == 0) {
            const unsigned xcc = __builtin_amdgcn_s_getreg((3 << 11) | 20) & 7u;
            atomicMax(&p.counters[12 + xcc], (unsigned long long)wall_clock64());
            atomicMax(&p.counters[20], ~t_start);
        }
    }
    if (COUNT) {
        unsigned long long sh = shortened;
        for (int off = 32; off > 0; off >>= 1) sh += __shfl_xor(sh, off);
        if (lane == 0) {
            if (sh) atomicAdd(&p.counters[9], sh);
            if (w_violations) atomicAdd(&p.counters[10], (unsigned long long)w_violations);
            if (w_verified) atomicAdd(&p.counters[21], (unsigned long long)w_verified);
        }
    }
    }
    if (!p.persist) break;
  }
}

static long long resident_workgroups(const void *func, size_t lds) {
    struct Key { const void *f; size_t lds; int dev; long long n; };
    static std::mutex mu;
    static std::vector<Key> cache;
    int dev = 0;
    if (hipGetDevice(&dev) != hipSuccess) { (void)hipGetLastError(); return 0; }
    std::lock_guard<std::mutex> lock(mu);
    for (const Key &k : cache) if (k.f == func && k.lds == lds && k.dev == dev) return k.n;
    int per_cu = 0;
    hipDeviceProp_t prop;
    long long n = 0;
    if (hipOccupancyMaxActiveBlocksPerMultiprocessor(&per_cu, func, HZ_TPB, lds) == hipSuccess && per_cu > 0 &&
        hipGetDeviceProperties(&prop, dev) == hipSuccess && prop.multiProcessorCount > 0)
        n = (long long)per_cu * prop.multiProcessorCount;
    else (void)hipGetLastError();
    cache.push_back(Key{func, lds, dev, n});
    return n;
}

template <int ALG, bool COUNT, bool STAGE, bool NODELET, bool LEVELSTACK>
static int launch_one(const HorizonParams &p_in, int grid, size_t lds, int persist_grid, hipStream_t st) {
    const void *func = reinterpret_cast<const void *>(k_horizon<ALG, COUNT, STAGE, NODELET, LEVELSTACK>);
    HZ_HIP(hipFuncSetAttribute(func, hipFuncAttributeMaxDynamicSharedMemorySize, (int)lds));
    HorizonParams p = p_in;
    if (p.persist) {
        const long long resident = persist_grid > 0 ? (long long)persist_grid : resident_workgroups(func, lds);
        if (resident <= 0 || (long long)grid <= resident) p.persist = 0;
        else {
            grid = (int)resident;
            HZ_HIP(hipMemsetAsync(p.queue, 0, 8 * sizeof(unsigned), st));
        }
    }
    hipLaunchKernelGGL((k_horizon<ALG, COUNT, STAGE, NODELET, LEVELSTACK>), dim3(grid), dim3(HZ_TPB), lds, st, p);
    HZ_HIP(hipGetLastError());
    return HZ_OK;
}

template <int ALG, bool STAGE, bool LS>
static int launch_left(const HorizonParams &p, size_t lds, int persist_grid, hipStream_t st) {
    const void *func = reinterpret_cast<const void *>(k_horizon<ALG, false, STAGE, false, LS, true>);
    HZ_HIP(hipFuncSetAttribute(func, hipFuncAttributeMaxDynamicSharedMemorySize, (int)lds));
    long long grid = p.tile_list ? (long long)((p.n_list + HZ_WPB - 1) / HZ_WPB)
                                 : (persist_grid > 0 ? (long long)persist_grid : resident_workgroups(func, lds));
    if (grid <= 0) grid = 1024;
    hipLaunchKernelGGL((k_horizon<ALG, false, STAGE, false, LS, true>), dim3((unsigned)grid), dim3(HZ_TPB), lds, st, p);
    HZ_HIP(hipGetLastError());
    return HZ_OK;
}

__device__ __forceinline__ unsigned hz_spread16(unsigned v) {
    v &= 0xffffu; v = (v | (v << 8)) & 0x00ff00ffu; v = (v | (v << 4)) & 0x0f0f0f0fu; v = (v | (v << 2)) & 0x33333333u; v = (v | (v << 1)) & 0x55555555u;
    return v;
}
__global__ __launch_bounds__(256) void k_left_keys(const unsigned *__restrict__ rec, unsigned cap, unsigned *__restrict__ ctl, unsigned dim_in_1,
                                                   unsigned azim_num, int morton_shift, int class_shift, unsigned *__restrict__ keys,
                                                   unsigned *__restrict__ vals) {
    const unsigned idx = blockIdx.x * 256u + threadIdx.x;
    const unsigned cnt = min(ctl[0], cap);
    bool valid = false;
    unsigned key = 0x00ffffffu;
    if (idx < cnt) {
        const unsigned c = rec[(size_t)idx * HZ_LEFT_WORDS];
        if (c != 0xffffffffu) {
            valid = true;
            const unsigned k = rec[(size_t)idx * HZ_LEFT_WORDS + 1];
            const unsigned r = min(azim_num > k ? azim_num - k : 0u, 511u);
            const unsigned di = c / dim_in_1, j = c - di * dim_in_1;
            const unsigned m = ((hz_spread16(di >> 4) << 1) | hz_spread16(j >> 4)) >> morton_shift;
            key = (((511u - r) >> class_shift) << 15) | (m & 0x7fffu);
        }
    }
    if (idx < cap) { keys[idx] = key; vals[idx] = idx; }
    const unsigned long long vm = __ballot(valid);
    if ((threadIdx.x & 63) == 0 && vm != 0ull) atomicAdd(&ctl[1], (unsigned)__popcll(vm));
}

int left_sort(const HorizonArgs &a, int r, hipStream_t st) {
    const unsigned cap = a.left_cap[r];
    if (cap == 0 || a.left_rec == nullptr || a.left_sort == nullptr) return HZ_OK;
    unsigned *ctl = reinterpret_cast<unsigned *>(a.counters + HZ_CNT_LEFT) + 16 * r;
    const int rows = a.row_end - a.row_begin;
    int bits = 0;
    while ((1 << bits) < std::max((rows + 15) / 16, (a.dim_in_1 + 15) / 16)) bits++;
    const int shift = std::max(0, 2 * bits - 15);
    uint32_t *ka = a.left_sort, *va = ka + a.left_cap_max, *kb = va + a.left_cap_max, *vb = kb + a.left_cap_max, *tmp = vb + a.left_cap_max;
    hipLaunchKernelGGL(k_left_keys, dim3((cap + 255u) / 256u), dim3(256), 0, st, a.left_rec + (size_t)a.left_base[r] * HZ_LEFT_WORDS, cap, ctl,
                       (unsigned)a.dim_in_1, (unsigned)a.azim_num, shift, a.left_key_shift, ka, va);
    HZ_HIP(hipGetLastError());
    return radix_sort_pairs_u32(ka, va, kb, vb, cap, tmp, st, 3);
}

template <int ALG>
static int launch_alg(const HorizonParams &p, int grid, size_t lds, bool count, bool level_stack, int pg, hipStream_t st) {
    const bool stage = p.stage_bytes != 0;
    if (p.left_mode) {
        if (level_stack) return stage ? launch_left<ALG, true, true>(p, lds, pg, st) : launch_left<ALG, false, true>(p, lds, pg, st);
        return stage ? launch_left<ALG, true, false>(p, lds, pg, st) : launch_left<ALG, false, false>(p, lds, pg, st);
    }
    if (ALG == ALG_GUESS && !count && p.top_nodes > 0) {
        if (!level_stack) return stage ? launch_one<ALG_GUESS, false, true, true, false>(p, grid, lds, pg, st)
                                       : launch_one<ALG_GUESS, false, false, true, false>(p, grid, lds, pg, st);
        return stage ? launch_one<ALG_GUESS, false, true, true, true>(p, grid, lds, pg, st)
                     : launch_one<ALG_GUESS, false, false, true, true>(p, grid, lds, pg, st);
    }
    if (level_stack) {
        if (count) return stage ? launch_one<ALG, true, true, false, true>(p, grid, lds, pg, st) : launch_one<ALG, true, false, false, true>(p, grid, lds, pg, st);
        return stage ? launch_one<ALG, false, true, false, true>(p, grid, lds, pg, st) : launch_one<ALG, false, false, false, true>(p, grid, lds, pg, st);
    }
    if (count) return stage ? launch_one<ALG, true, true, false, false>(p, grid, lds, pg, st) : launch_one<ALG, true, false, false, false>(p, grid, lds, pg, st);
    return stage ? launch_one<ALG, false, true, false, false>(p, grid, lds, pg, st) : launch_one<ALG, false, false, false, false>(p, grid, lds, pg, st);
}

int horizon_num_blocks(const HorizonArgs &a) {
    const int rows = a.row_end - a.row_begin;
    if (rows <= 0 || a.dim_in_1 <= 0) return 0;
    const TileMap tm = make_tile_map((rows + 15) / 16, (a.dim_in_1 + 15) / 16);
    return tm.per_xcd * 8 * 4;
}

int horizon_launch(const Scene *sc, const HorizonArgs &a, hipStream_t st, int *used_level_stack) {
    HorizonParams p;
    p.sv = scene_view(sc);
    p.tb.azim_sin = a.azim_sin; p.tb.azim_cos = a.azim_cos;
    p.tb.elev_ang = a.elev_ang; p.tb.elev_sin = a.elev_sin; p.tb.elev_cos = a.elev_cos; p.tb.mid_idx = a.mid_idx;
    p.tb.azim_num = a.azim_num; p.tb.elev_num = a.elev_num;
    p.tb.hori_acc = a.hori_acc; p.tb.low = a.low; p.tb.up = a.up;
    p.tb.step = (double)a.hori_acc / 5.0;
    p.vec_norm = a.vec_norm; p.vec_north = a.vec_north;
    p.mask = a.mask; p.hori = a.hori;
    p.offset_0 = a.offset_0; p.offset_1 = a.offset_1; p.dim_in_1 = a.dim_in_1;
    p.row_begin = a.row_begin; p.row_end = a.row_end;
    const int rows = a.row_end - a.row_begin;
    if (rows <= 0 || a.dim_in_1 <= 0) return HZ_OK;
    const int tiles_i = (rows + 15) / 16;
    p.tm = make_tile_map(tiles_i, (a.dim_in_1 + 15) / 16);
    p.dist = a.dist; p.hori_fill = a.hori_fill; p.ray_org_elev = a.ray_org_elev;
    p.dist_box = a.dist + 2.0f * p.sv.tau; p.neg_tau = -p.sv.tau;
    const int stage = ((a.azim_num & 3) == 0 && (reinterpret_cast<size_t>(a.hori) & 15) == 0) ? 4 * HZ_TPB * 4 : 0;
    const int pre = stage ? stage : 2 * HZ_TPB * 4;
    const int height = std::max(sc->hdr.height, 1);
    const int want_top = (a.top_nodes > 0 && a.alg == ALG_GUESS && !a.count_work) ? std::min(a.top_nodes, sc->hdr.n_top) : 0;
    const int lds_budget = 31 * 1024 / (4 / HZ_WPB);
    const int fast_cap = a.level_stack < 0 ? std::max(-a.level_stack, 4)
                                           : std::max((lds_budget - pre - want_top * (int)sizeof(Node)) / (HZ_TPB * 4), 4);
    const bool level_stack = a.level_stack > 0;
    const int depth = level_stack ? height : std::min(fast_cap, 3 * height + 1);
    if (used_level_stack) *used_level_stack = (level_stack || depth >= 3 * height + 1) ? 1 : 0;
    p.stack_cap = depth;
    p.stack_bytes = depth * HZ_TPB * 4;
    p.stage_bytes = stage;
    p.pre_bytes = pre;
    int top = (a.top_nodes > 0 && a.alg == ALG_GUESS && !a.count_work) ? a.top_nodes : 0;
    top = std::min(top, std::max(0, (80 * 1024 - (p.stack_bytes + p.pre_bytes)) / (int)sizeof(Node)));
    top = std::min(top, sc->hdr.n_top);
    p.top_nodes = top;
    p.regroup = (a.regroup <= 0) ? 36 : std::min(a.regroup & 0xff, 64);
    if (a.left_mode && a.left_regroup > 0) p.regroup = std::min(a.left_regroup, 64);
    p.leaf_bias = (a.regroup >= 256) ? (a.regroup >> 8) : 24;
    p.hit_cache = (a.hit_cache != 0) ? 1 : 0;
    p.near_idx = a.near_idx; p.near_r = a.near_r;
    p.verify_near = (a.verify_near > 0 && a.near_idx != nullptr) ? 1 : 0;
    p.scratch_row = a.count_work ? a.scratch_row : nullptr;
    {
        unsigned n = a.verify_near > 1 ? (unsigned)a.verify_near : 1u, m = 1u;
        while (m < n && m < (1u << 30)) m <<= 1;
        p.verify_mask = m - 1u;
    }
    p.counters = a.counters;
    p.tile_list = a.tile_list; p.n_list = a.n_list;
    p.redo_list = reinterpret_cast<int *>(a.counters + HZ_CNT_N);
    p.left_mode = std::max(a.left_mode, 0);
    p.left_rec = a.left_rec;
    unsigned *const left_ctl = reinterpret_cast<unsigned *>(a.counters + HZ_CNT_LEFT);
    const bool hands_over = a.left_rec != nullptr && !a.tile_list && !a.count_work && a.left_min > 0 && p.left_mode < HZ_LEFT_LEVELS &&
                            a.left_cap[p.left_mode] >= 64u;
    p.left_min = hands_over ? std::min(a.left_min, 56) : 0;
    p.left_in_base = p.left_mode ? a.left_base[p.left_mode - 1] : 0u;
    p.left_perm = (p.left_mode && a.left_sort) ? a.left_sort + 3 * a.left_cap_max : nullptr;
    p.left_in_ctl = left_ctl + 16 * (p.left_mode ? p.left_mode - 1 : 0);
    p.left_out_base = hands_over ? a.left_base[p.left_mode] : 0u;
    p.left_out_cap = hands_over ? a.left_cap[p.left_mode] : 0u;
    p.left_out_ctl = left_ctl + 16 * std::min(p.left_mode, HZ_LEFT_LEVELS - 1);
    p.persist = (a.tile_list == nullptr && ((!a.no_persist && HZ_WPB == 4) || p.left_mode)) ? 1 : 0;
    p.queue = reinterpret_cast<unsigned *>(a.counters + 24);
    const size_t lds = (size_t)p.pre_bytes + (size_t)p.stack_bytes + (size_t)top * sizeof(Node);
    const int grid = a.tile_list ? (a.n_list + HZ_WPB - 1) / HZ_WPB : p.tm.per_xcd * 8 * (4 / HZ_WPB);
    if (grid <= 0) return HZ_OK;
    const bool count = a.count_work != 0;
    int rc_launch;
    switch (a.alg) {
        case ALG_DISCRETE: rc_launch = launch_alg<ALG_DISCRETE>(p, grid, lds, count, level_stack, a.persist_grid, st); break;
        case ALG_BINARY: rc_launch = launch_alg<ALG_BINARY>(p, grid, lds, count, level_stack, a.persist_grid, st); break;
        default: rc_launch = launch_alg<ALG_GUESS>(p, grid, lds, count, level_stack, a.persist_grid, st); break;
    }
    return rc_launch;
}

__device__ __forceinline__ void hz_sincos_halfpi_f(float x, float &s, float &c) {
    const float y = 0.5f * x, z = y * y;
    float ps = 2.7557314e-06f;
    ps = ps * z + -1.9841270e-04f;
    ps = ps * z + 8.3333338e-03f;
    ps = ps * z + -1.6666667e-01f;
    float pc = -2.7557314e-07f;
    pc = pc * z + 2.4801587e-05f;
    pc = pc * z + -1.3888889e-03f;
    pc = pc * z + 4.1666668e-02f;
    const float sy = (y * z) * ps + y;
    const float cy = (z * z) * pc + (1.0f - 0.5f * z);
    s = (2.0f * sy) * cy;
    c = 1.0f - (2.0f * sy) * sy;
}

#define HZ_TOPO_CH 32
#ifndef HZ_TOPO_WG
#define HZ_TOPO_WG 3
#endif
template <int KIND>
__global__ __launch_bounds__(256, HZ_TOPO_WG) void k_topo(const float *__restrict__ azim, const float *__restrict__ hori,
                                             const float *__restrict__ vec_tilt, size_t ncell, int A,
                                             float *__restrict__ out) {
    extern __shared__ float topo_lds[];
    float *az_tab = topo_lds;
    const int wave = threadIdx.x >> 6, lane = threadIdx.x & 63;
    float *tile = topo_lds + 2 * A + wave * (64 * (HZ_TOPO_CH + 1));
    if (KIND != 2) {
        for (int k = threadIdx.x; k < A; k += blockDim.x) {
            az_tab[k] = (float)sin((double)azim[k]);
            az_tab[A + k] = (float)cos((double)azim[k]);
        }
    }
    const size_t cell0 = ((size_t)blockIdx.x * 4 + wave) * 64;
    const size_t c = cell0 + lane;
    const bool have = c < ncell;
    float tx = 0.0f, ty = 0.0f, tz = 1.0f;
    if (KIND != 2 && have) { tx = vec_tilt[3 * c]; ty = vec_tilt[3 * c + 1]; tz = vec_tilt[3 * c + 2]; }
    const float qx = -tx / tz, qy = -ty / tz;
    const double half_pi = 3.14159265358979323846 / 2.0;
    const float half_pi_f = 1.57079632679489661923f;
    float agg = 0.0f;
    const int half = lane >> 5, col = lane & 31;
    const size_t n_rows = cell0 < ncell ? min((size_t)64, ncell - cell0) : 0;
    const float *src = hori + (cell0 + half) * (size_t)A + col;
    float pre[32];
    auto fetch = [&](int k0) {
        const int n = min(HZ_TOPO_CH, A - k0);
#pragma unroll
        for (int r = 0; r < 32; r++) {
            pre[r] = 0.0f;
            if (col < n && (size_t)(2 * r + half) < n_rows) pre[r] = src[(size_t)(2 * r) * A + k0];
        }
    };
    fetch(0);
    __syncthreads();
    for (int k0 = 0; k0 < A; k0 += HZ_TOPO_CH) {
        const int n = min(HZ_TOPO_CH, A - k0);
        __builtin_amdgcn_fence(__ATOMIC_ACQ_REL, "wavefront");
        __builtin_amdgcn_wave_barrier();
#pragma unroll
        for (int r = 0; r < 32; r++) tile[(2 * r + half) * (HZ_TOPO_CH + 1) + col] = pre[r];
        if (k0 + HZ_TOPO_CH < A) fetch(k0 + HZ_TOPO_CH);
        __builtin_amdgcn_fence(__ATOMIC_ACQ_REL, "wavefront");
        __builtin_amdgcn_wave_barrier();
        if (!have) continue;
        const float *row = tile + lane * (HZ_TOPO_CH + 1);
#ifndef HZ_TOPO_UNROLL
#define HZ_TOPO_UNROLL 2
#endif
#pragma unroll HZ_TOPO_UNROLL
        for (int kk = 0; kk < n; kk++) {
            const float hv = row[kk];
            if (KIND == 2) {
                agg = (float)(((double)agg + half_pi) - (double)hv);
                continue;
            }
            const float as = az_tab[k0 + kk], ac = az_tab[A + k0 + kk];
            const float xf = as * qx + ac * qy;
            float sn, cs;
            hz_sincos_halfpi_f(hv, sn, cs);
            float he = hv;
            if (!(sn >= xf * cs)) {
                const float hp = atanf(xf);
                if (!(hv >= hp)) {
                    he = hp;
                    const float x2 = 1.0f + xf * xf;
                    const float rc = __builtin_amdgcn_rsqf(x2);
                    cs = rc; sn = (x2 == INFINITY) ? copysignf(1.0f, xf) : xf * rc;
                }
            }
            if (KIND == 0) {
                agg = agg + ((tx * as + ty * ac) * ((half_pi_f - he) - sn * cs) + tz * (cs * cs));
            } else {
                agg = agg + (1.0f - sn);
            }
        }
    }
    if (!have) return;
    if (KIND == 2) { out[c] = agg / (float)A; return; }
    const float azim_spac = azim[1] - azim[0];
    out[c] = (float)(((double)azim_spac / (2.0 * 3.14159265358979323846)) * (double)agg);
}

template <int KIND>
__global__ __launch_bounds__(256) void k_topo_wide(const float *__restrict__ azim, const float *__restrict__ hori,
                                                  const float *__restrict__ vec_tilt, size_t ncell, int A,
                                                  float *__restrict__ out) {
    const size_t c = (size_t)blockIdx.x * blockDim.x + threadIdx.x;
    if (c >= ncell) return;
    float tx = 0.0f, ty = 0.0f, tz = 1.0f;
    if (KIND != 2) { tx = vec_tilt[3 * c]; ty = vec_tilt[3 * c + 1]; tz = vec_tilt[3 * c + 2]; }
    const float *h = hori + c * (size_t)A;
    float agg = 0.0f;
    for (int k = 0; k < A; k++) {
        const float hv = h[k];
        if (KIND == 2) {
            agg = (float)(((double)agg + (3.14159265358979323846 / 2.0)) - (double)hv);
            continue;
        }
        const float as = (float)sin((double)azim[k]);
        const float ac = (float)cos((double)azim[k]);
        const float hori_plane = (float)atan((double)(-as * tx / tz - ac * ty / tz));
        const float he = (hv >= hori_plane) ? hv : hori_plane;
        if (KIND == 0) {
            const double ce = cos((double)he);
            agg = (float)((double)agg + ((double)(tx * as + ty * ac)
                          * ((3.14159265358979323846 / 2.0) - (double)he - (sin(2.0 * (double)he) / 2.0))
                          + (double)tz * (ce * ce)));
        } else {
            agg = (float)((double)agg + (1.0 - cos((3.14159265358979323846 / 2.0) - (double)he)));
        }
    }
    if (KIND == 2) { out[c] = agg / (float)A; return; }
    const float azim_spac = azim[1] - azim[0];
    out[c] = (float)(((double)azim_spac / (2.0 * 3.14159265358979323846)) * (double)agg);
}

#define HZ_TOPO_SVF 1
#define HZ_TOPO_VSF 2
#define HZ_TOPO_OPEN 4
template <int WANT>
__global__ __launch_bounds__(256, HZ_TOPO_WG) void k_topo_multi(const float *__restrict__ azim, const float *__restrict__ hori,
                                                   const float *__restrict__ vec_tilt, size_t ncell, int A,
                                                   float *__restrict__ out_svf, float *__restrict__ out_vsf,
                                                   float *__restrict__ out_open) {
    constexpr bool TILT = (WANT & (HZ_TOPO_SVF | HZ_TOPO_VSF)) != 0;
    extern __shared__ float topo_lds[];
// ... 174 lines not shown
```

### horayzon_amd/csrc/hz_internal.h

```cpp
#pragma once
#include <hip/hip_runtime.h>
#include <algorithm>
#include <chrono>
#include <cstdarg>
#include <cstdio>
#include <cstdlib>
#include "../../include/horayzon_hip.h"
#include "hz_common.h"
#include <atomic>
#include <mutex>

#define HZ_MAX_TOP_NODES 2047
#define HZ_MAX_STACK 40
#ifndef HZ_ANC_LEVELS
#define HZ_ANC_LEVELS 4
#endif

namespace hz {

int set_error(int code, const char *fmt, ...);

#define HZ_SHADOW_FAST_CAP_DEFAULT 19
extern std::atomic<int> g_shadow_fast_cap;
extern std::atomic<int> g_topo_wide;
extern std::atomic<int> g_accum_chunk;

#define HZ_HIP(expr)                                                                      \
    do {                                                                                  \
        hipError_t e_ = (expr);                                                           \
        if (e_ != hipSuccess)                                                             \
            return ::hz::set_error(HZ_ERR_HIP, "%s failed: %s (%s:%d)", #expr,            \
                                   hipGetErrorString(e_), __FILE__, __LINE__);            \
    } while (0)

struct Timer {
    std::chrono::high_resolution_clock::time_point t0;
    void start() { t0 = std::chrono::high_resolution_clock::now(); }
    double stop() const {
        return std::chrono::duration<double>(std::chrono::high_resolution_clock::now() - t0).count();
    }
};

struct Scene {
    int device = 0;
    hipStream_t stream = nullptr;
    void *blob = nullptr;
    size_t blob_bytes = 0;
    bool owns_blob = false;
    mutable std::atomic<int> level_stack{0};
    mutable std::mutex run_mu;
    mutable void *near_buf = nullptr;
    mutable size_t near_bytes = 0;
    mutable void *left_buf = nullptr;
    mutable size_t left_bytes = 0;
    BlobHeader hdr;
    const float *verts() const { return (const float *)((const char *)blob + hdr.off_verts); }
    const Node *nodes() const { return (const Node *)((const char *)blob + hdr.off_nodes); }
    const Prim *prims() const { return (const Prim *)((const char *)blob + hdr.off_prims); }
    const int *anc() const { return (const int *)((const char *)blob + hdr.off_anc); }
};

int scene_build(Scene *sc, const float *vert_grid, int d0, int d1, const float *vert_simp, int nvs,
                const int32_t *tri_simp, int nts, hz_stats *stats);

struct SceneView {
    const float *verts;
    const Node *nodes;
    const Prim *prims;
    const int *anc;
    int d1;
    int n_top;
    float cx, cy, cz;
    float tau;
};

inline SceneView scene_view(const Scene *sc) {
    SceneView v;
    v.verts = sc->verts(); v.nodes = sc->nodes(); v.prims = sc->prims(); v.anc = sc->anc();
    v.d1 = sc->hdr.d1; v.n_top = sc->hdr.n_top;
    v.cx = sc->hdr.center[0]; v.cy = sc->hdr.center[1]; v.cz = sc->hdr.center[2];
    v.tau = HZ_BOX_START_PADS * sc->hdr.pad;
    return v;
}

inline TileMap make_tile_map(int tiles_i, int tiles_j, int gw = 8) {
    TileMap m;
    m.tiles_i = tiles_i; m.tiles_j = tiles_j; m.gw = gw;
    m.rj = std::max(1, (tiles_j + 7) / 8);
    int pi = (tiles_i + m.rj - 1) / m.rj;
    pi = std::min(std::max(pi, std::min(16, tiles_i / 4)), 64);
    pi = std::max(1, std::min(pi, tiles_i));
    m.pi = pi;
    m.ri = (tiles_i + pi - 1) / pi;
    m.pi = (tiles_i + m.ri - 1) / m.ri;
    m.per_xcd = m.pi * m.ri * m.rj;
    return m;
}

bool is_device_ptr(const void *p);

#define HZ_LEFT_LEVELS 4
struct HorizonArgs {
    const float *vec_norm, *vec_north;
    const uint8_t *mask;
    float *hori;
    int offset_0, offset_1, dim_in_0, dim_in_1;
    int row_begin, row_end;
    int azim_num, elev_num, alg;
    float hori_acc, low, up, dist;
    float hori_fill, ray_org_elev;
    const float *azim_sin, *azim_cos, *elev_ang, *elev_sin, *elev_cos;
    const int *mid_idx;
    int top_nodes, regroup, count_work, hit_cache;
    int level_stack;
    const int *tile_list;
    int n_list;
    const unsigned short *near_idx;
    const float *near_r;
    int verify_near;
    float *scratch_row;
    int left_min = 0;
    unsigned *left_rec = nullptr;
    int left_mode = 0;
    unsigned left_base[HZ_LEFT_LEVELS] = {0, 0, 0, 0}, left_cap[HZ_LEFT_LEVELS] = {0, 0, 0, 0};
    int left_regroup = 0, left_key_shift = 0;
    uint32_t *left_sort = nullptr;
    unsigned left_cap_max = 0;
    int no_persist = 0;
    int persist_grid = 0;
    unsigned long long *counters;
};
#define HZ_LEFT_DEFAULT 0x00000024u
#define HZ_LEFT_KEY_SHIFT 3
#define HZ_LEFT_REGROUP 24
#define HZ_CNT_LEFT 32
#define HZ_CNT_N 64
#define HZ_LEFT_WORDS 16
#define HZ_REDO_CAP 16384
int horizon_launch(const Scene *sc, const HorizonArgs &a, hipStream_t st, int *used_level_stack = nullptr);
int left_sort(const HorizonArgs &a, int region, hipStream_t st);
int horizon_num_blocks(const HorizonArgs &a);
int topo_launch(int kind, const float *azim, const float *hori, const float *vec_tilt, int len_0, int len_1,
                int len_2, float *out, hipStream_t st);
int svf_launch(const float *azim, const float *hori, const float *vec_tilt, int len_0, int len_1,
               int len_2, float *svf, hipStream_t st);
int topo_multi_launch(const float *azim, const float *hori, const float *vec_tilt, int len_0, int len_1, int len_2,
                      float *svf, float *vsf, float *openness, hipStream_t st);

struct NearArgs {
    const float *vec_norm, *vec_north;
    const uint8_t *mask;
    const float *azim_sin, *azim_cos;
    int offset_0, offset_1, dim_in_1, row_begin, row_end, azim_num, elev_num;
    float ray_org_elev, hori_acc, low, up;
    unsigned short *near_idx;
    float *near_r;
    unsigned *reasons = nullptr;
    int ignore_bad_map = 0;
};
int near_launch(const Scene *sc, const NearArgs &a, hipStream_t st);
int near_max_azim();

struct LocationsArgs {
    const float *coords, *vec_norm, *vec_north, *ray_org_elev;
    float *hori, *dist;
    int num_loc, azim_num, elev_num, alg, hori_dist_out;
    float hori_acc, low, up, dist_m;
    const float *azim_sin, *azim_cos, *elev_ang, *elev_sin, *elev_cos;
    const int *mid_idx;
    unsigned long long *counters;
};
int locations_launch(const Scene *sc, const LocationsArgs &a, hipStream_t st);

struct ShadowArgs {
    const float *vec_tilt, *vec_norm, *surf_enl_fac, *elevation;
    const uint8_t *mask;
    int offset_0, offset_1, dim_in_0, dim_in_1;
    const float *suns;
    int num_sun;
    float sw_dir_cor_fill, dot_prod_min;
    int refrac_cor;
    const double *refrac_fac;
    int which;
    uint8_t *out_u8; float *out_f32;
    int top_nodes;
    int count_work;
    unsigned long long *counters;
};
int shadow_launch(const Scene *sc, const ShadowArgs &a, hipStream_t st);
int shadow_refrac_factor(const float *elevation, size_t n, double *out, hipStream_t st);
int accum_trace_launch(const Scene *sc, const ShadowArgs &a, int want_sw, hipStream_t st);
int accum_add_launch(const uint8_t *codes, const float *vals, size_t n, int k, const float *w, double *acc_sw, double *acc_lit,
                     hipStream_t st);
int accum_final_launch(const uint8_t *mask, size_t n, float fill, const double *acc_sw, const double *acc_lit, float *out_sw,
                       float *out_lit, hipStream_t st);

size_t sort_temp_elems(size_t n);
size_t scan_temp_elems(size_t n);
int radix_sort_pairs_u32(uint32_t *keys_a, uint32_t *vals_a, uint32_t *keys_b, uint32_t *vals_b, size_t n,
                         uint32_t *temp, hipStream_t st, int passes = 4);
int exclusive_scan_u32(const uint32_t *in, uint32_t *out, size_t n, uint32_t *temp, hipStream_t st);

#define HZ_COAST_LEAF 8
#define HZ_COAST_CNT_N 2
struct CoastIndex {
    uint32_t n_pts = 0, n_leaf = 0, n_leaf_pad = 1;
    size_t off_counters = 0, off_sorted = 0, off_nodes = 0, off_bbox = 0, off_sort = 0;
    unsigned long long *counters = nullptr;
    const double *sorted = nullptr;
    const void *nodes = nullptr;
};
size_t coast_scratch_bytes(size_t num_pts, CoastIndex *ix);
int coast_index_build(const double *pts, void *scratch, CoastIndex *ix, hipStream_t st);
int coast_query_launch(const CoastIndex &ix, const double *x, const double *y, const double *z, const uint8_t *mask_land,
                       int len_0, int len_1, int any_hit, double thr, double thr2, double *dist, uint8_t *mask_buffer,
                       hipStream_t st);

int bench_valu_peak(int packed, int waves_per_simd, double *winst_per_s_per_simd, double *clock_ghz, int *simds);
int bench_copy_peak(size_t bytes, double *gbs);
int bench_inst_rate(int op, double *cycles_per_inst);

int prep_slope(int which, const float *x, const float *y, const float *z, int len_0, int len_1,
               const float *rot_mat, int output_rot, float *vec_tilt, hipStream_t st);
int prep_lonlat2ecef(int ellps, const double *lon, const double *lat, const float *h, size_t n, double *X,
                     double *Y, double *Z, hipStream_t st);
int prep_ecef2enu(int ellps, double lon_or, double lat_or, const double *X, const double *Y, const double *Z,
                  size_t n, float *xe, float *ye, float *ze, hipStream_t st);
int prep_ecef2enu_vector(int ellps, double lon_or, double lat_or, const float *v, size_t n, float *o, hipStream_t st);
int prep_surf_norm(const double *lon, const double *lat, size_t n, float *o, hipStream_t st);
int prep_wgs2swiss(const double *lon, const double *lat, const float *h_wgs, size_t n, double *e, double *no, float *h_ch,
                   hipStream_t st);
int prep_swiss2wgs(const double *e, const double *no, const float *h_ch, size_t n, double *lon, double *lat, float *h_wgs,
                   hipStream_t st);
int prep_pack_vertices(const float *x, const float *y, const float *z, size_t n, size_t n_total, float *out,
                       hipStream_t st);
int prep_north_dir(int ellps, const double *X, const double *Y, const double *Z, const float *vn, size_t n,
                   float *o, hipStream_t st);

}
```

### horayzon_amd/csrc/hz_shadow.hip

```cpp
#include "hz_internal.h"
#include "hz_crmath.h"
#include <cstdlib>

namespace hz {

#define HZ_TPB 256
#ifndef HZ_SHADOW_LEAF_BIAS
#define HZ_SHADOW_LEAF_BIAS 24
#endif

struct ShadowParams {
    SceneView sv;
    const float *vec_tilt, *vec_norm, *surf_enl_fac, *elevation;
    const uint8_t *mask;
    int offset_0, offset_1, dim_in_0, dim_in_1;
    TileMap tm;
    const float *suns;
    size_t out_stride;
    float fill, dot_prod_min;
    int refrac, which;
    const double *refrac_fac;
    uint8_t *out_u8; float *out_f32;
    int top_nodes, stack_bytes;
    int stack_cap;
// ... 59 lines not shown
        }
        if (lane == 0) {
            atomicAdd(&p.counters[1], nc); atomicAdd(&p.counters[2], tn);
            atomicAdd(&p.counters[3], wn); atomicAdd(&p.counters[4], wl);
        }
    }
}

struct ShadowRay { float ox, oy, oz, dx, dy, dz, dot_ts, dot_ns; };

__device__ __forceinline__ int shadow_setup(const ShadowParams &p, int i, int j, float p_sun_x, float p_sun_y, float p_sun_z,
                                            uint8_t *out_u8, float *out_f32, ShadowRay &r) {
    const size_t cell = (size_t)i * p.dim_in_1 + j;
    if (p.mask[cell] != 1) {
        if (p.which == 0) out_u8[cell] = 3; else out_f32[cell] = p.fill;
        return 0;
    }
    const float tilt_x = p.vec_tilt[3 * cell], tilt_y = p.vec_tilt[3 * cell + 1], tilt_z = p.vec_tilt[3 * cell + 2];
    const float norm_x = p.vec_norm[3 * cell], norm_y = p.vec_norm[3 * cell + 1], norm_z = p.vec_norm[3 * cell + 2];
    const float ray_org_elev = 0.05f;
    const float *v = p.sv.verts + 3 * ((size_t)(i + p.offset_0) * p.sv.d1 + (size_t)(j + p.offset_1));
    const float ox = v[0] + norm_x * ray_org_elev;
    const float oy = v[1] + norm_y * ray_org_elev;
    const float oz = v[2] + norm_z * ray_org_elev;
    float sun_x = p_sun_x - ox, sun_y = p_sun_y - oy, sun_z = p_sun_z - oz;
    vec_unit(sun_x, sun_y, sun_z);
    float dot_prod_ns = (norm_x * sun_x + norm_y * sun_y) + norm_z * sun_z;
    if (p.refrac == 1) {
        const double fac = p.refrac_fac[cell];
        {
            const float dot0 = (tilt_x * sun_x + tilt_y * sun_y) + tilt_z * sun_z;
            const float tl = __builtin_fmaxf((tilt_x * tilt_x + tilt_y * tilt_y) + tilt_z * tilt_z, 1.0f);
            const float bound = (0.0114f * __builtin_fabsf((float)fac)) * tl * 1.01f + 1.0e-5f;
            if (dot0 < -bound) {
                if (p.which == 0) out_u8[cell] = 1; else out_f32[cell] = 0.0f;
                return 0;
            }
        }
        const float elev_ang_true = (float)(90.0 - (double)rad2deg_f(f_acos(dot_prod_ns)));
        const float refrac_cor = atmos_refrac(elev_ang_true, fac);
        float k_x = sun_y * norm_z - sun_z * norm_y;
        float k_y = sun_z * norm_x - sun_x * norm_z;
        float k_z = sun_x * norm_y - sun_y * norm_x;
        vec_unit(k_x, k_y, k_z);
        const float theta = deg2rad_f(refrac_cor);
        const float ct = f_cos(theta), st = f_sin(theta);
        const float part = (float)((double)((k_x * sun_x + k_y * sun_y) + k_z * sun_z) * (1.0 - (double)ct));
        const float rx = (sun_x * ct + (k_y * sun_z - k_z * sun_y) * st) + k_x * part;
        const float ry = (sun_y * ct + (k_z * sun_x - k_x * sun_z) * st) + k_y * part;
        const float rz = (sun_z * ct + (k_x * sun_y - k_y * sun_x) * st) + k_z * part;
        sun_x = rx; sun_y = ry; sun_z = rz;
        dot_prod_ns = (norm_x * sun_x + norm_y * sun_y) + norm_z * sun_z;
    }
    const float dot_prod_ts = (tilt_x * sun_x + tilt_y * sun_y) + tilt_z * sun_z;
    if (p.which == 0) {
        if (!(dot_prod_ts > 0.0f)) { out_u8[cell] = 1; return 0; }
    } else {
        if (!(dot_prod_ts > p.dot_prod_min)) { out_f32[cell] = 0.0f; return 0; }
    }
    r.ox = ox; r.oy = oy; r.oz = oz; r.dx = sun_x; r.dy = sun_y; r.dz = sun_z;
    r.dot_ts = dot_prod_ts; r.dot_ns = dot_prod_ns;
    return 1;
}

__device__ __forceinline__ void shadow_result(const ShadowParams &p, size_t cell, bool hit, const ShadowRay &r,
                                              uint8_t *out_u8, float *out_f32) {
    if (p.which == 0) { out_u8[cell] = hit ? 2 : 0; return; }
    if (hit) { out_f32[cell] = 0.0f; return; }
    float dot_prod_ns = r.dot_ns;
    if (dot_prod_ns < p.dot_prod_min) dot_prod_ns = p.dot_prod_min;
    out_f32[cell] = (r.dot_ts / dot_prod_ns) * p.surf_enl_fac[cell];
}


#ifndef HZ_SHADOW_FAST_CAP_DEFAULT
#define HZ_SHADOW_FAST_CAP_DEFAULT 19
#endif
#ifndef HZ_SHADOW_REGROUP
#define HZ_SHADOW_REGROUP 16
#endif
#ifndef HZ_SHADOW_WG
#define HZ_SHADOW_WG 7
#endif
template <bool COUNT, bool FAST>
__global__ __launch_bounds__(HZ_TPB, COUNT ? 5 : HZ_SHADOW_WG) void k_shadow_refill(ShadowParams p) {
    extern __shared__ __attribute__((aligned(16))) unsigned char smem[];
    int *stack = reinterpret_cast<int *>(smem + (FAST ? 2 * HZ_TPB * 4 : 0));
    const int tid = threadIdx.x;
    int ti = 0, tj = 0;
    const bool has_tile = hz_tile_of_block(p.tm, blockIdx.x, &ti, &tj);
    const int wave = tid >> 6, lane = tid & 63;
    const int sun_idx = blockIdx.y;
    const float p_sun_x = p.suns[3 * sun_idx], p_sun_y = p.suns[3 * sun_idx + 1], p_sun_z = p.suns[3 * sun_idx + 2];
    uint8_t *const out_u8 = p.out_u8 ? p.out_u8 + (size_t)sun_idx * p.out_stride : nullptr;
    float *const out_f32 = p.out_f32 ? p.out_f32 + (size_t)sun_idx * p.out_stride : nullptr;
    unsigned rays = 0;
    TravCounters tc; tc.nodes = 0; tc.tris = 0; tc.w_nodes = 0; tc.w_leaves = 0;
    const int i_base = ti * 16 + (wave >> 1) * 8, j_base = tj * (16 * p.nb) + (wave & 1) * 8;
    const int total = has_tile ? 64 * p.nb : 0;
    int next = 0;
    bool ray_active = false;
    ShadowRay r; r.ox = r.oy = r.oz = 0.0f; r.dx = r.dy = 0.0f; r.dz = 1.0f; r.dot_ts = r.dot_ns = 0.0f;
    size_t cell = 0;
    RayBox rb = hz_raybox(0, 0, 0, 0, 0, 1);
    TravState ts; hz_trav_reset(ts);
    bool overflow = false;
    for (;;) {
        if (next < total) {
            const unsigned long long need = __ballot(!ray_active);
            if (need != 0ull) {
                const int rank = __builtin_amdgcn_mbcnt_hi((unsigned)(need >> 32), __builtin_amdgcn_mbcnt_lo((unsigned)need, 0u));
                const int my = next + rank;
                next += __popcll(need);
                if (!ray_active && my < total) {
                    const int i = i_base + ((my & 63) >> 3), j = j_base + (my >> 6) * 16 + (my & 7);
                    if (i < p.dim_in_0 && j < p.dim_in_1 && shadow_setup(p, i, j, p_sun_x, p_sun_y, p_sun_z, out_u8, out_f32, r)) {
                        cell = (size_t)i * p.dim_in_1 + j;
                        rb = hz_raybox((r.ox - p.sv.cx) - p.sv.tau * r.dx, (r.oy - p.sv.cy) - p.sv.tau * r.dy, (r.oz - p.sv.cz) - p.sv.tau * r.dz,
                                       r.dx, r.dy, r.dz);
                        hz_trav_reset(ts);
                        overflow = false;
                        ray_active = true;
                        rays++;
                    }
                }
            }
        }
        if (__ballot(ray_active) == 0ull) {
            if (next >= total) break;
            continue;
        }
        if (ray_active) {
            int res = hz_trace<HZ_TPB, COUNT, 2, false, !FAST>(p.sv.nodes, p.sv.prims, nullptr, 0, stack, tid, r.ox, r.oy, r.oz, r.dx, r.dy, r.dz,
                                                    __builtin_inff(), __builtin_inff(), rb, ts, (next < total) ? HZ_SHADOW_REGROUP : 0, HZ_SHADOW_LEAF_BIAS, tc, p.stack_cap, overflow);
            if (FAST && res != 2 && overflow) {
                bool unused = false;
                hz_trav_reset(ts);
                res = hz_trace<HZ_TPB, COUNT, 2, false, true>(p.sv.nodes, p.sv.prims, nullptr, 0, stack, tid, r.ox, r.oy, r.oz, r.dx, r.dy, r.dz,
                                                                    __builtin_inff(), __builtin_inff(), rb, ts, 0, HZ_SHADOW_LEAF_BIAS, tc, 0, unused);
                if (COUNT && p.counters) atomicAdd(&p.counters[8], 1ull);
            }
            if (res != 2) {
                shadow_result(p, cell, res == 1, r, out_u8, out_f32);
                ray_active = false;
            }
        }
    }
    shadow_counters<COUNT>(p, rays, tc, lane);
}

std::atomic<int> g_shadow_fast_cap{HZ_SHADOW_FAST_CAP_DEFAULT};
std::atomic<int> g_topo_wide{0};
std::atomic<int> g_accum_chunk{0};

static int shadow_config(const Scene *sc, const ShadowArgs &a, ShadowParams &p, size_t &lds, dim3 &grid, bool &fast) {
    p.sv = scene_view(sc);
    p.vec_tilt = a.vec_tilt; p.vec_norm = a.vec_norm; p.surf_enl_fac = a.surf_enl_fac; p.elevation = a.elevation;
    p.mask = a.mask;
    p.offset_0 = a.offset_0; p.offset_1 = a.offset_1; p.dim_in_0 = a.dim_in_0; p.dim_in_1 = a.dim_in_1;
    if (a.dim_in_0 <= 0 || a.dim_in_1 <= 0) return 0;
    const int tiles_i = (a.dim_in_0 + 15) / 16;
    p.tm = make_tile_map(tiles_i, (a.dim_in_1 + 15) / 16);
    p.suns = a.suns; p.out_stride = (size_t)a.dim_in_0 * (size_t)a.dim_in_1;
    if (a.num_sun <= 0) return 0;
    p.fill = a.sw_dir_cor_fill; p.dot_prod_min = a.dot_prod_min;
    p.refrac = (a.refrac_cor && a.refrac_fac != nullptr) ? 1 : 0; p.which = a.which; p.refrac_fac = a.refrac_fac;
    p.out_u8 = a.out_u8; p.out_f32 = a.out_f32;
    p.stack_bytes = std::max(sc->hdr.height, 1) * HZ_TPB * 4;
    p.top_nodes = 0;
    p.counters = a.counters;
    const int fast_cap_env = g_shadow_fast_cap.load(std::memory_order_relaxed);
    const int height = std::max(sc->hdr.height, 1);
    const int fast_cap = std::min(fast_cap_env, 3 * height + 1);
    fast = fast_cap >= 5 && fast_cap >= height;
    p.stack_cap = fast ? fast_cap : 0;
    lds = fast ? (size_t)(fast_cap + 2) * HZ_TPB * 4 : (size_t)p.stack_bytes;
    {
        const int tiles_j = (a.dim_in_1 + 15) / 16;
        const double wgs = (double)tiles_i * tiles_j * (double)a.num_sun;
        int nb = (int)(wgs / (48.0 * 256.0));
        nb = std::max(1, std::min(std::min(nb, 32), tiles_j));
        for (int c = nb; c >= std::max(1, (nb * 3) / 4); c--)
            if (tiles_j % c == 0) { nb = c; break; }
        p.nb = nb;
        p.tm = make_tile_map(tiles_i, (tiles_j + nb - 1) / nb);
    }
    grid = dim3((unsigned)(p.tm.per_xcd * 8), (unsigned)a.num_sun);
    return 1;
}

#define HZ_LAUNCH_REFILL(K, P) do { \
        HZ_HIP(hipFuncSetAttribute(reinterpret_cast<const void *>(K), hipFuncAttributeMaxDynamicSharedMemorySize, (int)lds)); \
        hipLaunchKernelGGL(K, grid, dim3(HZ_TPB), lds, st, P); } while (0)

int shadow_launch(const Scene *sc, const ShadowArgs &a, hipStream_t st) {
    ShadowParams p;
    size_t lds = 0; dim3 grid; bool fast = false;
    if (!shadow_config(sc, a, p, lds, grid, fast)) return HZ_OK;
    if (fast) { if (a.count_work) HZ_LAUNCH_REFILL((k_shadow_refill<true, true>), p); else HZ_LAUNCH_REFILL((k_shadow_refill<false, true>), p); }
    else { if (a.count_work) HZ_LAUNCH_REFILL((k_shadow_refill<true, false>), p); else HZ_LAUNCH_REFILL((k_shadow_refill<false, false>), p); }
    HZ_HIP(hipGetLastError());
    return HZ_OK;
}

struct AccumParams {
    ShadowParams s;
    int want_sw;
};

__device__ __forceinline__ void accum_result(const AccumParams &p, size_t cell, bool hit, const ShadowRay &r,
                                             uint8_t *out_u8, float *out_f32) {
    if (p.s.which != 0) { shadow_result(p.s, cell, hit, r, out_u8, out_f32); return; }
    out_u8[cell] = hit ? 2 : 0;
    if (!p.want_sw || hit) return;
    float v = 0.0f;
    if (r.dot_ts > p.s.dot_prod_min) {
        float dot_prod_ns = r.dot_ns;
        if (dot_prod_ns < p.s.dot_prod_min) dot_prod_ns = p.s.dot_prod_min;
        v = (r.dot_ts / dot_prod_ns) * p.s.surf_enl_fac[cell];
    }
    out_f32[cell] = v;
}

template <bool COUNT, bool FAST>
__global__ __launch_bounds__(HZ_TPB, COUNT ? 5 : HZ_SHADOW_WG) void k_accum_refill(AccumParams ap) {
    const ShadowParams &p = ap.s;
    extern __shared__ __attribute__((aligned(16))) unsigned char smem[];
    int *stack = reinterpret_cast<int *>(smem + (FAST ? 2 * HZ_TPB * 4 : 0));
    const int tid = threadIdx.x;
    int ti = 0, tj = 0;
    const bool has_tile = hz_tile_of_block(p.tm, blockIdx.x, &ti, &tj);
    const int wave = tid >> 6, lane = tid & 63;
    const int sun_idx = blockIdx.y;
    const float p_sun_x = p.suns[3 * sun_idx], p_sun_y = p.suns[3 * sun_idx + 1], p_sun_z = p.suns[3 * sun_idx + 2];
    uint8_t *const out_u8 = p.out_u8 ? p.out_u8 + (size_t)sun_idx * p.out_stride : nullptr;
    float *const out_f32 = p.out_f32 ? p.out_f32 + (size_t)sun_idx * p.out_stride : nullptr;
    unsigned rays = 0;
    TravCounters tc; tc.nodes = 0; tc.tris = 0; tc.w_nodes = 0; tc.w_leaves = 0;
    const int i_base = ti * 16 + (wave >> 1) * 8, j_base = tj * (16 * p.nb) + (wave & 1) * 8;
    const int total = has_tile ? 64 * p.nb : 0;
    int next = 0;
    bool ray_active = false;
    ShadowRay r; r.ox = r.oy = r.oz = 0.0f; r.dx = r.dy = 0.0f; r.dz = 1.0f; r.dot_ts = r.dot_ns = 0.0f;
    size_t cell = 0;
    RayBox rb = hz_raybox(0, 0, 0, 0, 0, 1);
    TravState ts; hz_trav_reset(ts);
    bool overflow = false;
    for (;;) {
        if (next < total) {
            const unsigned long long need = __ballot(!ray_active);
            if (need != 0ull) {
                const int rank = __builtin_amdgcn_mbcnt_hi((unsigned)(need >> 32), __builtin_amdgcn_mbcnt_lo((unsigned)need, 0u));
                const int my = next + rank;
                next += __popcll(need);
                if (!ray_active && my < total) {
                    const int i = i_base + ((my & 63) >> 3), j = j_base + (my >> 6) * 16 + (my & 7);
                    if (i < p.dim_in_0 && j < p.dim_in_1 && shadow_setup(p, i, j, p_sun_x, p_sun_y, p_sun_z, out_u8, out_f32, r)) {
                        cell = (size_t)i * p.dim_in_1 + j;
                        rb = hz_raybox((r.ox - p.sv.cx) - p.sv.tau * r.dx, (r.oy - p.sv.cy) - p.sv.tau * r.dy, (r.oz - p.sv.cz) - p.sv.tau * r.dz,
                                       r.dx, r.dy, r.dz);
                        hz_trav_reset(ts);
                        overflow = false;
                        ray_active = true;
                        rays++;
                    }
                }
            }
        }
        if (__ballot(ray_active) == 0ull) {
            if (next >= total) break;
            continue;
        }
        if (ray_active) {
            int res = hz_trace<HZ_TPB, COUNT, 2, false, !FAST>(p.sv.nodes, p.sv.prims, nullptr, 0, stack, tid, r.ox, r.oy, r.oz, r.dx, r.dy, r.dz,
                                                    __builtin_inff(), __builtin_inff(), rb, ts, (next < total) ? HZ_SHADOW_REGROUP : 0, HZ_SHADOW_LEAF_BIAS, tc, p.stack_cap, overflow);
            if (FAST && res != 2 && overflow) {
                bool unused = false;
                hz_trav_reset(ts);
                res = hz_trace<HZ_TPB, COUNT, 2, false, true>(p.sv.nodes, p.sv.prims, nullptr, 0, stack, tid, r.ox, r.oy, r.oz, r.dx, r.dy, r.dz,
                                                                    __builtin_inff(), __builtin_inff(), rb, ts, 0, HZ_SHADOW_LEAF_BIAS, tc, 0, unused);
                if (COUNT && p.counters) atomicAdd(&p.counters[8], 1ull);
            }
            if (res != 2) {
                accum_result(ap, cell, res == 1, r, out_u8, out_f32);
                ray_active = false;
            }
        }
    }
    shadow_counters<COUNT>(p, rays, tc, lane);
}

int accum_trace_launch(const Scene *sc, const ShadowArgs &a, int want_sw, hipStream_t st) {
    AccumParams ap;
    size_t lds = 0; dim3 grid; bool fast = false;
    if (!shadow_config(sc, a, ap.s, lds, grid, fast)) return HZ_OK;
    ap.want_sw = want_sw;
    if (fast) { if (a.count_work) HZ_LAUNCH_REFILL((k_accum_refill<true, true>), ap); else HZ_LAUNCH_REFILL((k_accum_refill<false, true>), ap); }
    else { if (a.count_work) HZ_LAUNCH_REFILL((k_accum_refill<true, false>), ap); else HZ_LAUNCH_REFILL((k_accum_refill<false, false>), ap); }
    HZ_HIP(hipGetLastError());
    return HZ_OK;
}
#undef HZ_LAUNCH_REFILL

__global__ __launch_bounds__(256) void k_accum_add(const uint8_t *__restrict__ codes, const float *__restrict__ vals, size_t n,
                                                   int k, const float *__restrict__ w, double *__restrict__ acc_sw,
                                                   double *__restrict__ acc_lit) {
// ... 46 lines not shown
```

### horayzon_amd/horizon.py

```python
import ctypes as C

import numpy as np

from . import _lib
from . import _validate as V
from ._lib import Scene, hz_opts, hz_stats, hz_topo_out, ptr

TOPO_NAMES = ("svf", "vsf", "openness")
last_stats = None
schedule_overrides = {}


def _check_f32(a, ndim, name):
    if not isinstance(a, np.ndarray):
        raise TypeError("Argument '%s' has incorrect type (expected numpy.ndarray, got %s)"
                        % (name, type(a).__name__))
    if a.ndim != ndim:
        raise ValueError("Buffer has wrong number of dimensions (expected %d, got %d)" % (ndim, a.ndim))
    if a.dtype != np.float32:
        raise ValueError("Buffer dtype mismatch, expected 'float32_t' but got '%s'" % a.dtype.name)


def horizon_gridded(vert_grid, dem_dim_0, dem_dim_1, vec_norm, vec_north,
                    offset_0, offset_1, dist_search, azim_num=360, hori_acc=0.25,
                    ray_algorithm="guess_constant", geom_type="grid",
                    vert_simp=np.array([0.0, 0.0, 0.0, 0.0], dtype=np.float32),
                    num_vert_simp=1,
                    tri_ind_simp=np.array([0, 0, 0, 0], dtype=np.int32),
                    num_tri_simp=1, elev_ang_low_lim=-15.0, mask=None,
                    hori_fill=0.0, ray_org_elev=0.01, *, device=0, verbose=False,
                    scene=None, svf_vec_tilt=None, svf_only=False, rows=None, count_work=False, devices=None,
                    topo=None, topo_vec_tilt=None, topo_only=False,
                    _top_nodes=-1, _regroup=-1, _hit_cache=True, _chunk_rows=0, _near_skip=True, _level_stack=False,
                    _verify_near=False, _left_min=0, _persist_grid=0):
    global last_stats
    _check_f32(vert_grid, 1, "vert_grid")
    _check_f32(vec_norm, 3, "vec_norm")
    _check_f32(vec_north, 3, "vec_north")
    _check_f32(vert_simp, 1, "vert_simp")
    if not isinstance(tri_ind_simp, np.ndarray) or tri_ind_simp.ndim != 1 or tri_ind_simp.dtype != np.int32:
        raise ValueError("Buffer dtype mismatch, expected 'int32_t' for tri_ind_simp")
    if mask is not None and (not isinstance(mask, np.ndarray) or mask.ndim != 2):
        raise ValueError("Buffer has wrong number of dimensions (expected 2) for mask")

    if mask is None:
        mask = np.ones(vec_norm.shape[:2], dtype=np.uint8)
    V.run((
        (ValueError, "inconsistency between input arguments vert_grid, dem_dim_0 and dem_dim_1",
         lambda: not V.fits_grid(len(vert_grid), dem_dim_0, dem_dim_1)),
        (ValueError, "inconsistency between input arguments dem_dim_0, dem_dim_1, offset_0, offset_1 and vec_norm",
         lambda: not V.window_inside(offset_0, offset_1, vec_norm.shape, dem_dim_0, dem_dim_1)),
        (ValueError, V.MSG_NORTH, lambda: not V.same_leading_shape((vec_norm, vec_north), 3, 3)),
        (ValueError, V.MSG_ALG, lambda: ray_algorithm not in V.ALGORITHMS),
        (ValueError, V.MSG_GEOM, lambda: geom_type not in V.GEOMETRIES),
        (ValueError, "inconsistency between input arguments vert_simp and num_vert_simp", lambda: len(vert_simp) < num_vert_simp * 3),
        (ValueError, "inconsistency between input arguments tri_ind_simp and num_tri_simp", lambda: len(tri_ind_simp) < num_tri_simp * 3),
        (ValueError, "triangle indices of simplified outer domain exceed number of vertices",
         lambda: tri_ind_simp.max() > num_vert_simp - 1),
        (ValueError, V.MSG_ACC, lambda: hori_acc > 10.0),
        (ValueError, "shape of mask is inconsistent with other input", lambda: mask.shape[:2] != vec_norm.shape[:2]),
        (TypeError, V.MSG_MASK_TYPE, lambda: mask.dtype != "uint8"),
        (TypeError, V.MSG_ELEV, lambda: ray_org_elev < 0.005),
        (ValueError, V.MSG_DIM_LIMIT, lambda: max(dem_dim_0, dem_dim_1) > V.DIM_LIMIT),
        (ValueError, "vertex buffer vert_simp is larger than 16 GB", lambda: vert_simp.nbytes > 16.0e9),
    ))

    names = None if topo is None else ([topo] if isinstance(topo, str) else list(topo))
    tilted = names is not None and ("svf" in names or "vsf" in names)
    if topo_vec_tilt is not None:
        _check_f32(topo_vec_tilt, 3, "topo_vec_tilt")
    V.run((
        (ValueError, "'topo_only' needs 'topo'", lambda: topo_only and names is None),
        (ValueError, "'topo' cannot be combined with 'svf_vec_tilt' or 'svf_only' (ask for \"svf\" in 'topo')",
         lambda: names is not None and (svf_vec_tilt is not None or svf_only)),
        (ValueError, "'topo' is empty", lambda: names is not None and not names),
        (ValueError, "unknown name(s) in 'topo': %r (choose from %r)" % (
            [n for n in (names or ()) if n not in TOPO_NAMES], TOPO_NAMES),
         lambda: any(n not in TOPO_NAMES for n in names or ())),
        (ValueError, "'svf' and 'vsf' in 'topo' need 'topo_vec_tilt'", lambda: tilted and topo_vec_tilt is None),
        (ValueError, "'svf' and 'vsf' in 'topo' need azim_num >= 2", lambda: tilted and azim_num < 2),
        (ValueError, "shape of topo_vec_tilt is inconsistent with vec_norm",
         lambda: topo_vec_tilt is not None and topo_vec_tilt.shape != vec_norm.shape),
    ))

    vert_grid = np.ascontiguousarray(vert_grid)
    vec_norm = np.ascontiguousarray(vec_norm)
    vec_north = np.ascontiguousarray(vec_north)
    vert_simp = np.ascontiguousarray(vert_simp)
    tri_ind_simp = np.ascontiguousarray(tri_ind_simp)
    mask = np.ascontiguousarray(mask)

    dim_in_0, dim_in_1 = vec_norm.shape[0], vec_norm.shape[1]
    if svf_only and svf_vec_tilt is None:
        raise ValueError("'svf_only' needs 'svf_vec_tilt'")
    hori_buffer = None if (svf_only or topo_only) else np.empty((dim_in_0, dim_in_1, azim_num), dtype=np.float32)
    if rows is not None and hori_buffer is not None:
        hori_buffer.fill(np.nan)

    opts = hz_opts()
    opts.device = device
    opts.verbose = int(bool(verbose))
    opts.top_nodes = _top_nodes
    opts.regroup = _regroup
    opts.no_hit_cache = 0 if _hit_cache else 1
    opts.chunk_rows = _chunk_rows
    opts.no_near_skip = -1 if _near_skip == "force" else (0 if _near_skip else 1)
    opts.level_stack = int(_level_stack)
    opts.left_min = int(_left_min or schedule_overrides.get("left_min", 0))
    opts.persist_grid = int(_persist_grid or schedule_overrides.get("persist_grid", 0))
    opts.left_cap_test = int(schedule_overrides.get("left_cap_test", 0))
    opts.left_tune = int(schedule_overrides.get("left_tune", 0))
    n_verify = int(_verify_near)
    if n_verify < 0 or n_verify != _verify_near:
        raise ValueError("_verify_near must be a non-negative integer (or a bool)")
    opts.verify_near = n_verify
    opts.skip_hori = 1 if (svf_only or topo_only) else 0
    opts.count_work = int(bool(count_work))
    if rows is not None:
        if len(rows) != 2 or not (0 <= int(rows[0]) < int(rows[1]) <= dim_in_0):
            raise ValueError("'rows' must be (begin, end) with 0 <= begin < end <= %d" % dim_in_0)
        opts.row_begin, opts.row_end = int(rows[0]), int(rows[1])
    svf = None
    if svf_vec_tilt is not None:
        _check_f32(svf_vec_tilt, 3, "svf_vec_tilt")
        if azim_num < 2:
            raise ValueError("sky view factor needs azim_num >= 2")
        if svf_vec_tilt.shape != vec_norm.shape:
            raise ValueError("Inconsistent/incorrect shapes of input arrays")
        svf_vec_tilt = np.ascontiguousarray(svf_vec_tilt)
        svf = np.full((dim_in_0, dim_in_1), np.nan, dtype=np.float32)
        opts.svf = ptr(svf)
        opts.vec_tilt = ptr(svf_vec_tilt)
    maps, topo_out = None, None
    if names is not None:
        maps = {n: np.full((dim_in_0, dim_in_1), np.nan, dtype=np.float32) for n in TOPO_NAMES if n in names}
        if tilted:
            topo_vec_tilt = np.ascontiguousarray(topo_vec_tilt)
            opts.vec_tilt = ptr(topo_vec_tilt)
        if "svf" in maps:
            opts.svf = ptr(maps["svf"])
        if "vsf" in maps or "openness" in maps:
            topo_out = hz_topo_out(ptr(maps.get("vsf")), ptr(maps.get("openness")))
    stats = hz_stats()
    L = _lib.lib()

    def run(o, st):
        ex = () if topo_out is None else (C.byref(topo_out),)
        if scene is None:
            return (L.hz_horizon_gridded_ex if ex else L.hz_horizon_gridded)(
                ptr(vert_grid), dem_dim_0, dem_dim_1, ptr(vec_norm), ptr(vec_north),
                offset_0, offset_1, ptr(hori_buffer), dim_in_0, dim_in_1, azim_num,
                dist_search, hori_acc, ray_algorithm.encode("utf-8"),
                geom_type.encode("utf-8"), ptr(vert_simp), num_vert_simp,
                ptr(tri_ind_simp), num_tri_simp, elev_ang_low_lim, ptr(mask),
                hori_fill, ray_org_elev, C.byref(o), *ex, C.byref(st))
        o.device = scene.device
        return (L.hz_horizon_gridded_scene_ex if ex else L.hz_horizon_gridded_scene)(
            scene._h, ptr(vec_norm), ptr(vec_north), offset_0, offset_1,
            ptr(hori_buffer), dim_in_0, dim_in_1, azim_num, dist_search, hori_acc,
            ray_algorithm.encode("utf-8"), elev_ang_low_lim, ptr(mask), hori_fill,
            ray_org_elev, C.byref(o), *ex, C.byref(st))

    if devices is None:
        rc = run(opts, stats)
    else:
        import threading
        from .dist import row_slabs
        if scene is not None or rows is not None:
            raise ValueError("'devices' cannot be combined with 'scene' or 'rows'")
        devs = list(range(_lib.device_count())) if isinstance(devices, str) and devices == "all" \
            else [int(d) for d in devices]
        if not devs:
            raise ValueError("'devices' is empty")
        slabs = [sl for sl in row_slabs(mask, len(devs))]
        part, errs = [None] * len(devs), []

        def work(idx):
            b, e = slabs[idx]
            if e <= b:
                return
            o = hz_opts.from_buffer_copy(opts)
            o.device, o.row_begin, o.row_end = devs[idx], b, e
            st = hz_stats()
            try:
                _lib.check(run(o, st))
                part[idx] = st
            except Exception as exc:
                errs.append(exc)
        threads = [threading.Thread(target=work, args=(i,)) for i in range(len(devs))]
        for t in threads:
            t.start()
        for t in threads:
            t.join()
        if errs:
            raise errs[0]
        for st in part:
            if st is None:
                continue
            for name, _ in hz_stats._fields_:
                a, b = getattr(stats, name), getattr(st, name)
                setattr(stats, name, max(a, b) if name.startswith("t_") or name in ("bvh_height", "elev_num", "scene_bytes") else a + b)
        rc = 0
    _lib.check(rc)
    last_stats = stats.as_dict()

    azim = np.empty(azim_num, dtype=np.float32)
    for i in range(azim_num):
        azim[i] = ((2 * np.pi) / azim_num * i)

    if maps is not None:
        return hori_buffer, azim, maps
    if svf is not None:
        return hori_buffer, azim, svf
    return hori_buffer, azim


def horizon_locations(vert_grid, dem_dim_0, dem_dim_1, coords, vec_norm, vec_north,
                      dist_search, azim_num=360, hori_acc=0.25,
                      ray_algorithm="binary_search", geom_type="grid",
                      elev_ang_low_lim=-89.98,
                      ray_org_elev=np.array([0.01], dtype=np.float32),
                      hori_dist_out=False, *, device=0, verbose=False, scene=None):
    global last_stats
    _check_f32(vert_grid, 1, "vert_grid")
    _check_f32(coords, 2, "coords")
    _check_f32(vec_norm, 2, "vec_norm")
    _check_f32(vec_north, 2, "vec_north")
    _check_f32(ray_org_elev, 1, "ray_org_elev")

    V.run((
        (ValueError, "inconsistency between input arguments vert_grid, dem_dim_0 and dem_dim_1",
         lambda: not V.fits_grid(len(vert_grid), dem_dim_0, dem_dim_1)),
        (ValueError, "'number of dimensions and/or dimension length(s) of 'coords' incorrect",
         lambda: coords.ndim != 2 or coords.shape != (vec_norm.shape[0], 3)),
        (ValueError, V.MSG_NORTH, lambda: not V.same_leading_shape((vec_norm, vec_north), 2, 2)),
        (ValueError, V.MSG_ALG, lambda: ray_algorithm not in V.ALGORITHMS),
        (ValueError, V.MSG_GEOM, lambda: geom_type not in V.GEOMETRIES),
        (ValueError, V.MSG_ACC, lambda: hori_acc > 10.0),
        (ValueError, "length of array 'ray_org_elev' must be either one or correspond to the number of locations",
         lambda: len(ray_org_elev) not in (1, coords.shape[0])),
        (TypeError, V.MSG_ELEV, lambda: ray_org_elev.min() < 0.005),
        (TypeError, "horizon detection algorithm 'guess_constant' not implemented for horizon distance computation",
         lambda: bool(hori_dist_out) and ray_algorithm == "guess_constant"),
        (ValueError, V.MSG_DIM_LIMIT, lambda: max(dem_dim_0, dem_dim_1) > V.DIM_LIMIT),
    ))

    if len(ray_org_elev) != coords.shape[0]:
        ray_org_elev = np.repeat(ray_org_elev, coords.shape[0])

    vert_grid = np.ascontiguousarray(vert_grid)
    coords = np.ascontiguousarray(coords)
    vec_norm = np.ascontiguousarray(vec_norm)
    vec_north = np.ascontiguousarray(vec_north)
    ray_org_elev = np.ascontiguousarray(ray_org_elev)

    num_loc = vec_norm.shape[0]
    hori_buffer = np.empty((num_loc, azim_num), dtype=np.float32)
    hori_buffer.fill(np.nan)
    hori_dist_buffer = np.empty((num_loc if hori_dist_out else 1, azim_num), dtype=np.float32)
    hori_dist_buffer.fill(np.nan)

    opts = hz_opts()
    opts.device = device if scene is None else scene.device
    opts.verbose = int(bool(verbose))
    stats = hz_stats()
    L = _lib.lib()
    if num_loc == 0:
        rc = 0
    elif scene is None:
        rc = L.hz_horizon_locations(
            ptr(vert_grid), dem_dim_0, dem_dim_1, ptr(coords), ptr(vec_norm), ptr(vec_north),
            ptr(hori_buffer), ptr(hori_dist_buffer) if hori_dist_out else None, num_loc, azim_num,
            dist_search, hori_acc, ray_algorithm.encode("utf-8"), geom_type.encode("utf-8"),
            elev_ang_low_lim, ptr(ray_org_elev), int(bool(hori_dist_out)), C.byref(opts), C.byref(stats))
    else:
        rc = L.hz_horizon_locations_scene(
            scene._h, ptr(coords), ptr(vec_norm), ptr(vec_north), ptr(hori_buffer),
            ptr(hori_dist_buffer) if hori_dist_out else None, num_loc, azim_num, dist_search, hori_acc,
            ray_algorithm.encode("utf-8"), elev_ang_low_lim, ptr(ray_org_elev), int(bool(hori_dist_out)),
            C.byref(opts), C.byref(stats))
    _lib.check(rc)
    last_stats = stats.as_dict()

    azim = np.empty(azim_num, dtype=np.float32)
    for i in range(azim_num):
        azim[i] = ((2 * np.pi) / azim_num * i)

    if hori_dist_out:
        return hori_buffer, hori_dist_buffer, azim
    else:
        return hori_buffer, azim


def horizon_tables(azim_num, hori_acc, elev_ang_low_lim):
    L = _lib.lib()
    n = C.c_int(0)
    _lib.check(L.hz_horizon_tables(azim_num, hori_acc, elev_ang_low_lim, None, None, 0,
# ... 9 lines not shown
```

Measured before the change: 9.929 million.

## Split persistent horizon queue tail onto low-priority stream to overlap leftover drain

Splits the persistent work queue of each horizon chunk into a head part on the main stream and a tail part (about one resident wave of blocks) launched on a separate low-priority stream. The tail has its own queue counter, leftover region, sort buffer and redo list, so the main stream's leftover sort and drain can overlap with the tail's execution instead of waiting behind the straggling tail of the main kernel. The aim is to fill the GPU idle time during the drain phase. The cost is extra launches, events, cross-stream synchronisation, more leftover buffer memory and an additional overflow/redo path.

```diff
diff --git a/horayzon_amd/csrc/hz_api.hip b/horayzon_amd/csrc/hz_api.hip
--- a/horayzon_amd/csrc/hz_api.hip
+++ b/horayzon_amd/csrc/hz_api.hip
@@ -133,28 +133,34 @@
 }
 
 static std::mutex g_stream_mu;
-static std::vector<std::pair<int, hipStream_t>> g_stream_pool;
-
-static int stream_acquire(int device, hipStream_t *st) {
+static std::vector<std::pair<int, hipStream_t>> g_stream_pool[2];
+
+static int stream_acquire(int device, hipStream_t *st, bool low_priority = false) {
+    std::vector<std::pair<int, hipStream_t>> &pool = g_stream_pool[low_priority ? 1 : 0];
     {
         std::lock_guard<std::mutex> lk(g_stream_mu);
-        for (size_t i = 0; i < g_stream_pool.size(); i++)
-            if (g_stream_pool[i].first == device) {
-                *st = g_stream_pool[i].second;
-                g_stream_pool.erase(g_stream_pool.begin() + (long)i);
+        for (size_t i = 0; i < pool.size(); i++)
+            if (pool[i].first == device) {
+                *st = pool[i].second;
+                pool.erase(pool.begin() + (long)i);
                 return HZ_OK;
             }
     }
-    const hipError_t e = hipStreamCreateWithFlags(st, hipStreamNonBlocking);
+    hipError_t e;
+    if (low_priority) {
+        int least = 0, greatest = 0;
+        if (hipDeviceGetStreamPriorityRange(&least, &greatest) != hipSuccess) { (void)hipGetLastError(); least = 0; }
+        e = hipStreamCreateWithPriority(st, hipStreamNonBlocking, least);
+    } else e = hipStreamCreateWithFlags(st, hipStreamNonBlocking);
     if (e != hipSuccess) return set_error(HZ_ERR_HIP, "hipStreamCreate failed: %s", hipGetErrorString(e));
     return HZ_OK;
 }
 
-static void stream_release(int device, hipStream_t st) {
+static void stream_release(int device, hipStream_t st, bool low_priority = false) {
     if (!st) return;
     (void)hipStreamSynchronize(st);
     std::lock_guard<std::mutex> lk(g_stream_mu);
-    g_stream_pool.emplace_back(device, st);
+    g_stream_pool[low_priority ? 1 : 0].emplace_back(device, st);
 }
 
 static int scene_new(int device, Scene **out) {
@@ -440,7 +446,9 @@
     return rc;
 }
 
-static int plan_leftover(const Scene *sc, const hz_opts *opts, int rows_max, int dim_in_1, int left_t[HZ_LEFT_LEVELS], HorizonArgs &a) {
+static int plan_leftover(const Scene *sc, const hz_opts *opts, int rows_max, int dim_in_1, int left_t[HZ_LEFT_LEVELS], HorizonArgs &a,
+                         unsigned long long tail_units, uint32_t **sort2, unsigned *cap2) {
+    *sort2 = nullptr; *cap2 = 0u;
     int n_left_launches = 0;
     for (int l = 0; l < HZ_LEFT_LEVELS; l++) left_t[l] = 0;
     const int pack = opts ? opts->left_min : 0;
@@ -461,9 +469,17 @@
         total += cap; cap_max = std::max(cap_max, cap);
         units = cap / 64ull;
     }
+    unsigned long long cap_tail = 0;
+    if (tail_units > 0 && n_left_launches == 1) {
+        cap_tail = ((tail_units * (unsigned long long)left_t[0] + 63ull) & ~63ull) + 64ull;
+        if (opts && opts->left_cap_test > 0) cap_tail = std::min<unsigned long long>(cap_tail, ((unsigned long long)opts->left_cap_test + 63ull) & ~63ull);
+        a.left_base[1] = (unsigned)total; a.left_cap[1] = (unsigned)cap_tail;
+        total += cap_tail;
+    }
     const size_t rec_bytes = (size_t)total * HZ_LEFT_WORDS * sizeof(unsigned);
     const size_t sort_words = 4 * (size_t)cap_max + sort_temp_elems((size_t)cap_max) + 64;
-    const size_t need = rec_bytes + sort_words * sizeof(uint32_t);
+    const size_t sort2_words = cap_tail ? 4 * (size_t)cap_tail + sort_temp_elems((size_t)cap_tail) + 64 : 0;
+    const size_t need = rec_bytes + (sort_words + sort2_words) * sizeof(uint32_t);
     if (total >= (1ull << 31) || (unsigned long long)rows_max * (unsigned long long)dim_in_1 >= 0xffffffffull) return 0;
     if (sc->left_bytes < need) {
         if (sc->left_buf) (void)hipFree(sc->left_buf);
@@ -472,6 +488,7 @@
         sc->left_bytes = need;
     }
     a.left_sort = (uint32_t *)((char *)sc->left_buf + rec_bytes); a.left_cap_max = (unsigned)cap_max;
+    if (cap_tail) { *sort2 = a.left_sort + sort_words; *cap2 = (unsigned)cap_tail; }
     return n_left_launches;
 }
 
@@ -575,7 +592,7 @@
     DevIn<unsigned long long> d_cnt;
     unsigned long long zeros[HZ_CNT_N] = {0};
     void *cnt_dev = nullptr;
-    HZ_HIP(hipMalloc(&cnt_dev, sizeof(zeros) + 2 * HZ_REDO_CAP * sizeof(int)));
+    HZ_HIP(hipMalloc(&cnt_dev, sizeof(zeros) + HZ_REDO_LISTS * HZ_REDO_CAP * sizeof(int)));
     d_cnt.owned = cnt_dev;
     HZ_HIP(hipStreamSynchronize(st));
     const double h2d_s = t_h2d.stop();
@@ -610,10 +627,11 @@
     int fallbacks = 0;
     unsigned long long redo_blocks = 0, redo_groups = 0;
 
-    struct Ev { hipEvent_t a = nullptr, b = nullptr, c = nullptr, d = nullptr, l = nullptr; };
+    struct Ev { hipEvent_t a = nullptr, b = nullptr, c = nullptr, d = nullptr, l = nullptr, cert = nullptr, tail = nullptr; };
     std::vector<Ev> evs;
     std::vector<size_t> ev_of;
     hipStream_t st_copy = nullptr;
+    hipStream_t st_tail = nullptr;
     auto free_events = [&]() {
         for (auto &e : evs) {
             if (e.a) (void)hipEventDestroy(e.a);
@@ -621,8 +639,11 @@
             if (e.c) (void)hipEventDestroy(e.c);
             if (e.d) (void)hipEventDestroy(e.d);
             if (e.l) (void)hipEventDestroy(e.l);
+            if (e.cert) (void)hipEventDestroy(e.cert);
+            if (e.tail) (void)hipEventDestroy(e.tail);
         }
         if (st_copy) { stream_release(sc->device, st_copy); st_copy = nullptr; }
+        if (st_tail) { stream_release(sc->device, st_tail, true); st_tail = nullptr; }
     };
     if (stream_out && (rc = stream_acquire(sc->device, &st_copy))) return rc;
     if (use_near) {
@@ -635,14 +656,39 @@
             sc->near_bytes = need;
         }
     }
+    a.persist_grid = (opts && opts->persist_grid > 0) ? opts->persist_grid : 0;
+    a.no_persist = (opts && opts->persist_grid < 0) ? 1 : 0;
+    const int split_opt = g_drain_split.load(std::memory_order_relaxed);
+    const bool split_allowed = split_opt >= 0 && !(opts && opts->count_work) && verify_n == 0;
+    auto split_tail = [&](const HorizonArgs &ha, int *n_out) -> int {
+        long long resident = 0;
+        if (!split_allowed || horizon_launch(sc, ha, st, nullptr, &resident) != HZ_OK || resident <= 0) return 0;
+        const long long n = (long long)horizon_num_blocks(ha) / 8;
+        if (n < 2 * resident) return 0;
+        const long long f = split_opt > 0 ? (n * (long long)std::min(split_opt, 1000) + 999) / 1000 : resident;
+        *n_out = (int)n;
+        return (int)std::max<long long>(1, std::min(f, n - 1));
+    };
+    unsigned long long tail_units = 0;
+    if (split_allowed) {
+        HorizonArgs ha = a;
+        ha.level_stack = (sc->level_stack.load(std::memory_order_relaxed) != 0 || (opts && opts->level_stack > 0)) ? 1
+                         : ((opts && opts->level_stack < 0) ? opts->level_stack : 0);
+        ha.row_begin = row_begin; ha.row_end = row_begin + std::min(chunk_rows, row_end - row_begin);
+        ha.hori = (skip_hori || stream_out) ? (float *)tmp_hori : d_hori.dev;
+        if (ha.hori) ha.hori -= (size_t)ha.row_begin * dim_in_1 * azim_num;
+        int n_q = 0;
+        tail_units = 8ull * (unsigned long long)split_tail(ha, &n_q);
+    }
+    uint32_t *left_sort2 = nullptr;
+    unsigned left_cap2 = 0;
     int left_t[HZ_LEFT_LEVELS];
-    const int n_left_launches = plan_leftover(sc, opts, std::min(chunk_rows, row_end - row_begin), dim_in_1, left_t, a);
+    const int n_left_launches = plan_leftover(sc, opts, std::min(chunk_rows, row_end - row_begin), dim_in_1, left_t, a, tail_units, &left_sort2, &left_cap2);
+    bool chunk_split = false;
     a.left_min = n_left_launches > 0 ? left_t[0] : 0;
     a.left_rec = n_left_launches > 0 ? (unsigned *)sc->left_buf : nullptr;
     a.left_regroup = (opts && (opts->left_tune & 0xff) > 0) ? (opts->left_tune & 0xff) : HZ_LEFT_REGROUP;
     a.left_key_shift = (opts && ((opts->left_tune >> 8) & 0xff) > 0) ? std::min(((opts->left_tune >> 8) & 0xff) - 1, 8) : HZ_LEFT_KEY_SHIFT;
-    a.persist_grid = (opts && opts->persist_grid > 0) ? opts->persist_grid : 0;
-    a.no_persist = (opts && opts->persist_grid < 0) ? 1 : 0;
     unsigned *near_reasons = nullptr;
     struct ReasonsFree { unsigned **p; ~ReasonsFree() { if (*p) (void)hipFree(*p); } } reasons_free{&near_reasons};
     if (use_near && opts && opts->verbose >= 2) {
@@ -676,7 +722,13 @@
             return set_error(HZ_ERR_HIP, "copy of the horizon chunk failed: %s", hipGetErrorString(hipGetLastError()));
         return HZ_OK;
     };
-    auto fail = [&](int code) { (void)hipStreamSynchronize(st); if (st_copy) (void)hipStreamSynchronize(st_copy); free_events(); return code; };
+    auto fail = [&](int code) {
+        (void)hipStreamSynchronize(st);
+        if (st_tail) (void)hipStreamSynchronize(st_tail);
+        if (st_copy) (void)hipStreamSynchronize(st_copy);
+        free_events();
+        return code;
+    };
     int n_chunk = 0;
     unsigned long long left_cells = 0, left_again = 0;
     float ms_left = 0.0f;
@@ -718,7 +770,45 @@
             if (verify_n > 0 && !a.count_work && use_near) {
                 if ((rc = mon.launch(sc, a, verify_n, rb, st))) return fail(rc);
             }
+            auto launch_split = [&](int f, int n_q, int *safe_out) -> int {
+                Ev &ev = evs.back();
+                HorizonArgs h = a, t = a;
+                h.q_begin = 0; h.q_end = n_q - f;
+                t.q_begin = n_q - f; t.q_end = n_q; t.queue_set = 1; t.left_out = 1;
+                HZ_HIP(hipEventRecord(ev.cert, st));
+                HZ_HIP(hipStreamWaitEvent(st_tail, ev.cert, 0));
+                int r = horizon_launch(sc, h, st, safe_out);
+                if (r) return r;
+                chunk_split = true;
+                if (!(r = horizon_launch(sc, t, st_tail, nullptr))) {
+                    (void)hipEventRecord(ev.l, st);
+                    HorizonArgs b = a;
+                    b.left_mode = 1; b.left_min = 0; b.tile_list = nullptr; b.n_list = 0;
+                    if (!(r = left_sort(a, 0, st))) r = horizon_launch(sc, b, st, nullptr);
+                    if (!r) {
+                        HorizonArgs b2 = a;
+                        b2.left_sort = left_sort2; b2.left_cap_max = left_cap2;
+                        b2.left_mode = 2; b2.left_min = 0; b2.tile_list = nullptr; b2.n_list = 0;
+                        if (!(r = left_sort(b2, 1, st_tail))) r = horizon_launch(sc, b2, st_tail, nullptr);
+                    }
+                }
+                HZ_HIP(hipEventRecord(ev.tail, st_tail));
+                HZ_HIP(hipStreamWaitEvent(st, ev.tail, 0));
+                return r;
+            };
             auto launch_chunk = [&](int *safe_out) -> int {
+                chunk_split = false;
+                if (n_left_launches == 1 && left_sort2 != nullptr && !a.tile_list) {
+                    int n_q = 0;
+                    const int f = split_tail(a, &n_q);
+                    bool ok = f > 0 && 8ull * (unsigned long long)f <= tail_units;
+                    if (ok && !st_tail && stream_acquire(sc->device, &st_tail, true) != HZ_OK) { (void)hipGetLastError(); st_tail = nullptr; ok = false; }
+                    Ev &ev = evs.back();
+                    if (ok && !ev.l && hipEventCreate(&ev.l) != hipSuccess) { (void)hipGetLastError(); ev.l = nullptr; ok = false; }
+                    if (ok && !ev.cert && hipEventCreateWithFlags(&ev.cert, hipEventDisableTiming) != hipSuccess) { (void)hipGetLastError(); ev.cert = nullptr; ok = false; }
+                    if (ok && !ev.tail && hipEventCreateWithFlags(&ev.tail, hipEventDisableTiming) != hipSuccess) { (void)hipGetLastError(); ev.tail = nullptr; ok = false; }
+                    if (ok) return launch_split(f, n_q, safe_out);
+                }
                 int r = horizon_launch(sc, a, st, safe_out);
                 if (r || n_left_launches == 0) return r;
                 if (!evs.back().l && hipEventCreate(&evs.back().l) != hipSuccess) return set_error(HZ_ERR_HIP, "hipEventCreate failed");
@@ -740,13 +830,13 @@
                 if (hipMemcpyAsync(cov, cnt_dev, sizeof(cov), hipMemcpyDeviceToHost, st) != hipSuccess ||
                     hipStreamSynchronize(st) != hipSuccess)
                     return fail(set_error(HZ_ERR_HIP, "horizon kernel failed: %s", hipGetErrorString(hipGetLastError())));
-                const unsigned long long ov = cov[8], lov = cov[30];
-                if (ov != 0 || lov != 0) {
+                const unsigned long long ov = cov[8], lov = cov[30], lov1 = chunk_split ? cov[31] : 0ull;
+                if (ov != 0 || lov != 0 || lov1 != 0) {
                     const unsigned long long tiles = (unsigned long long)((re - rb + 7) / 8) * (unsigned long long)((dim_in_1 + 7) / 8);
                     fallbacks++;
                     a.level_stack = 1;
-                    if (ov <= HZ_REDO_CAP && lov <= HZ_REDO_CAP && (ov + lov) * 4 <= tiles) {
-                        redo_blocks += ov + lov; redo_groups += lov;
+                    if (ov <= HZ_REDO_CAP && lov <= HZ_REDO_CAP && lov1 <= HZ_REDO_CAP && (ov + lov + lov1) * 4 <= tiles) {
+                        redo_blocks += ov + lov + lov1; redo_groups += lov + lov1;
                         if (ov != 0) {
                             a.tile_list = reinterpret_cast<const int *>((unsigned long long *)cnt_dev + HZ_CNT_N);
                             a.n_list = (int)ov;
@@ -758,6 +848,14 @@
                             b.left_mode = 1; b.left_min = 0;
                             b.tile_list = reinterpret_cast<const int *>((unsigned long long *)cnt_dev + HZ_CNT_N) + HZ_REDO_CAP;
                             b.n_list = (int)lov;
+                            rc = horizon_launch(sc, b, st, nullptr);
+                        }
+                        if (!rc && lov1 != 0) {
+                            HorizonArgs b = a;
+                            b.left_sort = left_sort2; b.left_cap_max = left_cap2;
+                            b.left_mode = 2; b.left_min = 0;
+                            b.tile_list = reinterpret_cast<const int *>((unsigned long long *)cnt_dev + HZ_CNT_N) + 2 * HZ_REDO_CAP;
+                            b.n_list = (int)lov1;
                             rc = horizon_launch(sc, b, st, nullptr);
                         }
                     } else {
@@ -1263,6 +1361,7 @@
     if (!strcmp(key, "shadow_fast_cap")) hz::g_shadow_fast_cap.store(value < 0 ? HZ_SHADOW_FAST_CAP_DEFAULT : value, std::memory_order_relaxed);
     else if (!strcmp(key, "topo_wide")) hz::g_topo_wide.store(value != 0, std::memory_order_relaxed);
     else if (!strcmp(key, "accum_chunk")) hz::g_accum_chunk.store(value < 0 ? 0 : value, std::memory_order_relaxed);
+    else if (!strcmp(key, "drain_split")) hz::g_drain_split.store(value < 0 ? -1 : std::min(value, 1000), std::memory_order_relaxed);
     else return hz::set_error(HZ_ERR_ARG, "hz_debug_set: unknown key '%s'", key);
     return HZ_OK;
 }
diff --git a/horayzon_amd/csrc/hz_horizon.hip b/horayzon_amd/csrc/hz_horizon.hip
--- a/horayzon_amd/csrc/hz_horizon.hip
+++ b/horayzon_amd/csrc/hz_horizon.hip
@@ -119,7 +119,7 @@
             int q = 0;
             if (lane == 0) q = (int)atomicAdd(&p.queue[x], 1u);
             q = __builtin_amdgcn_readfirstlane(q);
-            if (q < p.tm.per_xcd * 4) { blk = (((q >> 2) * 8 + x) << 2) | (q & 3); break; }
+            if (q < p.n_list) { blk = (((q >> 2) * 8 + x) << 2) | (q & 3); break; }
             xcc_off++;
         }
         if (blk < 0) break;
@@ -333,8 +333,9 @@
     const bool wave_overflowed = !LEVELSTACK && __ballot(overflow) != 0ull;
     if (wave_overflowed) {
         if (lane == 0) {
-            const unsigned long long slot = atomicAdd(&p.counters[LEFT ? 30 : 8], 1ull);
-            if (slot < (unsigned long long)HZ_REDO_CAP) p.redo_list[(LEFT ? HZ_REDO_CAP : 0) + (int)slot] = blk;
+            const int set = (LEFT && p.left_mode == 2) ? 1 : 0;
+            const unsigned long long slot = atomicAdd(&p.counters[LEFT ? 30 + set : 8], 1ull);
+            if (slot < (unsigned long long)HZ_REDO_CAP) p.redo_list[(LEFT ? (1 + set) * HZ_REDO_CAP : 0) + (int)slot] = blk;
         }
     } else {
     const int guard_cells = __popcll(__ballot(guards != 0u && !(LEFT && had_guard)));
@@ -388,16 +389,24 @@
 }
 
 template <int ALG, bool COUNT, bool STAGE, bool NODELET, bool LEVELSTACK>
-static int launch_one(const HorizonParams &p_in, int grid, size_t lds, int persist_grid, hipStream_t st) {
+static int launch_one(const HorizonParams &p_in, int grid, size_t lds, int persist_grid, int q_begin, hipStream_t st, long long *resident_query) {
     const void *func = reinterpret_cast<const void *>(k_horizon<ALG, COUNT, STAGE, NODELET, LEVELSTACK>);
     HZ_HIP(hipFuncSetAttribute(func, hipFuncAttributeMaxDynamicSharedMemorySize, (int)lds));
     HorizonParams p = p_in;
+    if (resident_query) {
+        const long long resident = !p.persist ? 0 : (persist_grid > 0 ? (long long)persist_grid : resident_workgroups(func, lds));
+        *resident_query = (resident > 0 && (long long)grid > resident) ? resident : 0;
+        return HZ_OK;
+    }
     if (p.persist) {
         const long long resident = persist_grid > 0 ? (long long)persist_grid : resident_workgroups(func, lds);
-        if (resident <= 0 || (long long)grid <= resident) p.persist = 0;
+        if (resident <= 0 || (long long)grid <= resident) {
+            if (q_begin != 0 || p.n_list != p.tm.per_xcd * 4) return set_error(HZ_ERR_ARG, "a queue window needs a persistent launch");
+            p.persist = 0; p.n_list = 0;
+        }
         else {
             grid = (int)resident;
-            HZ_HIP(hipMemsetAsync(p.queue, 0, 8 * sizeof(unsigned), st));
+            HZ_HIP(hipMemsetD32Async(reinterpret_cast<hipDeviceptr_t>(p.queue), q_begin, 8, st));
         }
     }
     hipLaunchKernelGGL((k_horizon<ALG, COUNT, STAGE, NODELET, LEVELSTACK>), dim3(grid), dim3(HZ_TPB), lds, st, p);
@@ -460,24 +469,25 @@
 }
 
 template <int ALG>
-static int launch_alg(const HorizonParams &p, int grid, size_t lds, bool count, bool level_stack, int pg, hipStream_t st) {
+static int launch_alg(const HorizonParams &p, int grid, size_t lds, bool count, bool level_stack, int pg, int qb, hipStream_t st, long long *rq) {
     const bool stage = p.stage_bytes != 0;
     if (p.left_mode) {
+        if (rq) { *rq = 0; return HZ_OK; }
         if (level_stack) return stage ? launch_left<ALG, true, true>(p, lds, pg, st) : launch_left<ALG, false, true>(p, lds, pg, st);
         return stage ? launch_left<ALG, true, false>(p, lds, pg, st) : launch_left<ALG, false, false>(p, lds, pg, st);
     }
     if (ALG == ALG_GUESS && !count && p.top_nodes > 0) {
-        if (!level_stack) return stage ? launch_one<ALG_GUESS, false, true, true, false>(p, grid, lds, pg, st)
-                                       : launch_one<ALG_GUESS, false, false, true, false>(p, grid, lds, pg, st);
-        return stage ? launch_one<ALG_GUESS, false, true, true, true>(p, grid, lds, pg, st)
-                     : launch_one<ALG_GUESS, false, false, true, true>(p, grid, lds, pg, st);
+        if (!level_stack) return stage ? launch_one<ALG_GUESS, false, true, true, false>(p, grid, lds, pg, qb, st, rq)
+                                       : launch_one<ALG_GUESS, false, false, true, false>(p, grid, lds, pg, qb, st, rq);
+        return stage ? launch_one<ALG_GUESS, false, true, true, true>(p, grid, lds, pg, qb, st, rq)
+                     : launch_one<ALG_GUESS, false, false, true, true>(p, grid, lds, pg, qb, st, rq);
     }
     if (level_stack) {
-        if (count) return stage ? launch_one<ALG, true, true, false, true>(p, grid, lds, pg, st) : launch_one<ALG, true, false, false, true>(p, grid, lds, pg, st);
-        return stage ? launch_one<ALG, false, true, false, true>(p, grid, lds, pg, st) : launch_one<ALG, false, false, false, true>(p, grid, lds, pg, st);
-    }
-    if (count) return stage ? launch_one<ALG, true, true, false, false>(p, grid, lds, pg, st) : launch_one<ALG, true, false, false, false>(p, grid, lds, pg, st);
-    return stage ? launch_one<ALG, false, true, false, false>(p, grid, lds, pg, st) : launch_one<ALG, false, false, false, false>(p, grid, lds, pg, st);
+        if (count) return stage ? launch_one<ALG, true, true, false, true>(p, grid, lds, pg, qb, st, rq) : launch_one<ALG, true, false, false, true>(p, grid, lds, pg, qb, st, rq);
+        return stage ? launch_one<ALG, false, true, false, true>(p, grid, lds, pg, qb, st, rq) : launch_one<ALG, false, false, false, true>(p, grid, lds, pg, qb, st, rq);
+    }
+    if (count) return stage ? launch_one<ALG, true, true, false, false>(p, grid, lds, pg, qb, st, rq) : launch_one<ALG, true, false, false, false>(p, grid, lds, pg, qb, st, rq);
+    return stage ? launch_one<ALG, false, true, false, false>(p, grid, lds, pg, qb, st, rq) : launch_one<ALG, false, false, false, false>(p, grid, lds, pg, qb, st, rq);
 }
 
 int horizon_num_blocks(const HorizonArgs &a) {
@@ -487,7 +497,8 @@
     return tm.per_xcd * 8 * 4;
 }
 
-int horizon_launch(const Scene *sc, const HorizonArgs &a, hipStream_t st, int *used_level_stack) {
+int horizon_launch(const Scene *sc, const HorizonArgs &a, hipStream_t st, int *used_level_stack, long long *resident_query) {
+    if (resident_query) *resident_query = 0;
     HorizonParams p;
     p.sv = scene_view(sc);
     p.tb.azim_sin = a.azim_sin; p.tb.azim_cos = a.azim_cos;
@@ -541,26 +552,30 @@
     p.left_mode = std::max(a.left_mode, 0);
     p.left_rec = a.left_rec;
     unsigned *const left_ctl = reinterpret_cast<unsigned *>(a.counters + HZ_CNT_LEFT);
-    const bool hands_over = a.left_rec != nullptr && !a.tile_list && !a.count_work && a.left_min > 0 && p.left_mode < HZ_LEFT_LEVELS &&
-                            a.left_cap[p.left_mode] >= 64u;
+    const int out_region = a.left_out >= 0 ? std::min(a.left_out, HZ_LEFT_LEVELS - 1) : p.left_mode;
+    const bool hands_over = a.left_rec != nullptr && !a.tile_list && !a.count_work && a.left_min > 0 && out_region < HZ_LEFT_LEVELS &&
+                            a.left_cap[out_region] >= 64u;
     p.left_min = hands_over ? std::min(a.left_min, 56) : 0;
     p.left_in_base = p.left_mode ? a.left_base[p.left_mode - 1] : 0u;
     p.left_perm = (p.left_mode && a.left_sort) ? a.left_sort + 3 * a.left_cap_max : nullptr;
     p.left_in_ctl = left_ctl + 16 * (p.left_mode ? p.left_mode - 1 : 0);
-    p.left_out_base = hands_over ? a.left_base[p.left_mode] : 0u;
-    p.left_out_cap = hands_over ? a.left_cap[p.left_mode] : 0u;
-    p.left_out_ctl = left_ctl + 16 * std::min(p.left_mode, HZ_LEFT_LEVELS - 1);
+    p.left_out_base = hands_over ? a.left_base[out_region] : 0u;
+    p.left_out_cap = hands_over ? a.left_cap[out_region] : 0u;
+    p.left_out_ctl = left_ctl + 16 * std::min(out_region, HZ_LEFT_LEVELS - 1);
+
     p.persist = (a.tile_list == nullptr && ((!a.no_persist && HZ_WPB == 4) || p.left_mode)) ? 1 : 0;
-    p.queue = reinterpret_cast<unsigned *>(a.counters + 24);
+    p.queue = reinterpret_cast<unsigned *>(a.counters + (a.queue_set ? HZ_CNT_QUEUE2 : 24));
+    const int q_begin = a.q_end > 0 ? std::max(a.q_begin, 0) : 0;
+    if (p.persist && !p.left_mode) p.n_list = a.q_end > 0 ? std::min(a.q_end, p.tm.per_xcd * 4) : p.tm.per_xcd * 4;
     const size_t lds = (size_t)p.pre_bytes + (size_t)p.stack_bytes + (size_t)top * sizeof(Node);
     const int grid = a.tile_list ? (a.n_list + HZ_WPB - 1) / HZ_WPB : p.tm.per_xcd * 8 * (4 / HZ_WPB);
     if (grid <= 0) return HZ_OK;
     const bool count = a.count_work != 0;
     int rc_launch;
     switch (a.alg) {
-        case ALG_DISCRETE: rc_launch = launch_alg<ALG_DISCRETE>(p, grid, lds, count, level_stack, a.persist_grid, st); break;
-        case ALG_BINARY: rc_launch = launch_alg<ALG_BINARY>(p, grid, lds, count, level_stack, a.persist_grid, st); break;
-        default: rc_launch = launch_alg<ALG_GUESS>(p, grid, lds, count, level_stack, a.persist_grid, st); break;
+        case ALG_DISCRETE: rc_launch = launch_alg<ALG_DISCRETE>(p, grid, lds, count, level_stack, a.persist_grid, q_begin, st, resident_query); break;
+        case ALG_BINARY: rc_launch = launch_alg<ALG_BINARY>(p, grid, lds, count, level_stack, a.persist_grid, q_begin, st, resident_query); break;
+        default: rc_launch = launch_alg<ALG_GUESS>(p, grid, lds, count, level_stack, a.persist_grid, q_begin, st, resident_query); break;
     }
     return rc_launch;
 }
diff --git a/horayzon_amd/csrc/hz_internal.h b/horayzon_amd/csrc/hz_internal.h
--- a/horayzon_amd/csrc/hz_internal.h
+++ b/horayzon_amd/csrc/hz_internal.h
@@ -23,6 +23,7 @@
 #define HZ_SHADOW_FAST_CAP_DEFAULT 19
 extern std::atomic<int> g_shadow_fast_cap;
 extern std::atomic<int> g_topo_wide;
+extern std::atomic<int> g_drain_split;
 extern std::atomic<int> g_accum_chunk;
 
 #define HZ_HIP(expr)                                                                      \
@@ -127,6 +128,8 @@
     uint32_t *left_sort = nullptr;
     unsigned left_cap_max = 0;
     int no_persist = 0;
+    int q_begin = 0, q_end = 0, queue_set = 0;
+    int left_out = -1;
     int persist_grid = 0;
     unsigned long long *counters;
 };
@@ -134,10 +137,12 @@
 #define HZ_LEFT_KEY_SHIFT 3
 #define HZ_LEFT_REGROUP 24
 #define HZ_CNT_LEFT 32
-#define HZ_CNT_N 64
+#define HZ_CNT_QUEUE2 64
+#define HZ_CNT_N 72
+#define HZ_REDO_LISTS 3
 #define HZ_LEFT_WORDS 16
 #define HZ_REDO_CAP 16384
-int horizon_launch(const Scene *sc, const HorizonArgs &a, hipStream_t st, int *used_level_stack = nullptr);
+int horizon_launch(const Scene *sc, const HorizonArgs &a, hipStream_t st, int *used_level_stack = nullptr, long long *resident_query = nullptr);
 int left_sort(const HorizonArgs &a, int region, hipStream_t st);
 int horizon_num_blocks(const HorizonArgs &a);
 int topo_launch(int kind, const float *azim, const float *hori, const float *vec_tilt, int len_0, int len_1,
diff --git a/horayzon_amd/csrc/hz_shadow.hip b/horayzon_amd/csrc/hz_shadow.hip
--- a/horayzon_amd/csrc/hz_shadow.hip
+++ b/horayzon_amd/csrc/hz_shadow.hip
@@ -235,6 +235,7 @@
 std::atomic<int> g_shadow_fast_cap{HZ_SHADOW_FAST_CAP_DEFAULT};
 std::atomic<int> g_topo_wide{0};
 std::atomic<int> g_accum_chunk{0};
+std::atomic<int> g_drain_split{0};
 
 static int shadow_config(const Scene *sc, const ShadowArgs &a, ShadowParams &p, size_t &lds, dim3 &grid, bool &fast) {
     p.sv = scene_view(sc);
diff --git a/horayzon_amd/horizon.py b/horayzon_amd/horizon.py
--- a/horayzon_amd/horizon.py
+++ b/horayzon_amd/horizon.py
@@ -32,7 +32,7 @@
                     scene=None, svf_vec_tilt=None, svf_only=False, rows=None, count_work=False, devices=None,
                     topo=None, topo_vec_tilt=None, topo_only=False,
                     _top_nodes=-1, _regroup=-1, _hit_cache=True, _chunk_rows=0, _near_skip=True, _level_stack=False,
-                    _verify_near=False, _left_min=0, _persist_grid=0):
+                    _verify_near=False, _left_min=0, _persist_grid=0, _drain_split=0):
     global last_stats
     _check_f32(vert_grid, 1, "vert_grid")
     _check_f32(vec_norm, 3, "vec_norm")
@@ -143,6 +143,7 @@
             topo_out = hz_topo_out(ptr(maps.get("vsf")), ptr(maps.get("openness")))
     stats = hz_stats()
     L = _lib.lib()
+    _lib.check(L.hz_debug_set(b"drain_split", int(_drain_split or schedule_overrides.get("drain_split", 0))))
 
     def run(o, st):
         ex = () if topo_out is None else (C.byref(topo_out),)
```

Result: no change. 9.968 million (median of 6 runs) (+0.4%).
